# maruscia/fastkmer

Hardware: AMD Instinct MI355X
Metric: input bases/sec (whole node), k=28 short reads, 1/2/4/8 GPUs (higher is better)
Workload: dtype u64; 1 GPU; BASELINE configs[1]: k=28 m=10 x=3 B=2048, 1 GB synthetic 100 bp reads per GPU; k=28, m=10, x=3, B=2048, useHT=0, sequenceType=0, fasta_bytes_per_gpu=999999906, bases_per_gpu=877192900, parallelism=one GPU

## Files before the change

fastkmer_amd/__init__.py:

```python
from __future__ import annotations

import ctypes
import dataclasses
import os
import re

import numpy as np

_PKG = os.path.dirname(os.path.abspath(__file__))
LIB_PATH = os.environ.get("FASTKMER_LIB") or os.path.join(_PKG, "lib", "libfastkmer.so")
CLI_PATH = os.path.join(_PKG, "bin", "fastkmer-cli")
HEADER_PATH = os.path.join(os.path.dirname(_PKG), "include", "fastkmer.h")

FK_OK = 0
ERRORS = {-1: "FK_E_INVALID", -2: "FK_E_STATE", -3: "FK_E_DEVICE", -4: "FK_E_NOMEM", -5: "FK_E_IO",
          -6: "FK_E_RANGE", -7: "FK_E_COMM"}
ABI_VERSION = 3


class FastKmerError(RuntimeError):
    def __init__(self, code: int, message: str):
        super().__init__(f"{ERRORS.get(code, code)}: {message}")
        self.code = code

# ... 74 lines not shown
        "fk_synth_record_bytes": (U64, [I32]),
        "fk_synth_fasta_host": (ctypes.c_int, [P, U64, U64, I32, U64, U64, ctypes.c_double, ctypes.c_double]),
        "fk_create": (ctypes.c_int, [ctypes.POINTER(fk_config), ctypes.POINTER(P)]),
        "fk_destroy": (None, [P]),
        "fk_last_error": (ctypes.c_char_p, []),
        "fk_set_stream": (ctypes.c_int, [P, P]),
        "fk_ingest": (ctypes.c_int, [P, ctypes.c_char_p, SZ, ctypes.c_int]),
        "fk_ingest_device": (ctypes.c_int, [P, P, SZ, ctypes.c_int]),
        "fk_ingest_reserve": (ctypes.c_int, [P, U64]),
        "fk_split_bytes": (ctypes.c_int, [ctypes.c_char_p, I32, I32, I32, I32, P, SZ, ctypes.POINTER(SZ)]),
        "fk_ingest_file_range": (ctypes.c_int, [P, ctypes.c_char_p, I32, I32, U64]),
        "fk_set_input_format": (ctypes.c_int, [P, I32, I32, I32]),
        "fk_input_format": (ctypes.c_int, [P, ctypes.POINTER(I32), ctypes.POINTER(I32), ctypes.POINTER(I32)]),
        "fk_fastq_info": (ctypes.c_int, [P, P]),
        "fk_debug_fastq_ms": (ctypes.c_int, [P, ctypes.POINTER(ctypes.c_double), ctypes.POINTER(U64)]),
        "fk_fastq_frontier": (ctypes.c_int, [ctypes.c_char_p, SZ, ctypes.POINTER(SZ)]),
        "fk_split_bytes_fastq": (ctypes.c_int, [ctypes.c_char_p, I32, I32, P, SZ, ctypes.POINTER(SZ)]),
        "fk_synth_fasta_device": (ctypes.c_int, [P, U64, U64, I32, U64, U64, ctypes.c_double, ctypes.c_double]),
        "fk_synth_fasta_to_device": (ctypes.c_int, [P, U64, U64, I32, U64, U64, ctypes.c_double, ctypes.c_double]),
        "fk_map": (ctypes.c_int, [P, P]),
        "fk_record_bytes": (SZ, [P]),
        "fk_map_emit": (ctypes.c_int, [P, P, U64]),
        "fk_reduce": (ctypes.c_int, [P, P, U64]),
        "fk_set_grouped_emit": (ctypes.c_int, [P, ctypes.c_int32]),
        "fk_grouped_parts_per_rank": (ctypes.c_int32, [P]),
        "fk_map_part_counts": (ctypes.c_int, [P, P, P]),
        "fk_reduce_grouped": (ctypes.c_int, [P, P, U64, P, P, ctypes.c_int32, ctypes.c_int32]),
        "fk_finish": (ctypes.c_int, [P]),
        "fk_num_bins": (I32, [P]),
        "fk_bin_sizes": (ctypes.c_int, [P, P]),
        "fk_get_bin": (ctypes.c_int, [P, I32, P, P, SZ, ctypes.POINTER(SZ)]),
        "fk_write_bins": (ctypes.c_int, [P, ctypes.c_char_p]),
        "fk_get_stats": (ctypes.c_int, [P, ctypes.POINTER(fk_stats)]),
        "fk_kmer_bin": (ctypes.c_int, [ctypes.POINTER(fk_config), P, P]),
        "fk_query": (ctypes.c_int, [P, P, SZ, P, P]),
        "fk_query_device": (ctypes.c_int, [P, P, SZ, P, P]),
        "fk_query_sequence": (ctypes.c_int, [P, ctypes.c_char_p, SZ, P, SZ, ctypes.POINTER(SZ)]),
        "fk_reads_csr": (ctypes.c_int, [ctypes.c_char_p, SZ, I32, I32, I32, P, SZ, P, SZ, ctypes.POINTER(SZ),
                                        ctypes.POINTER(SZ)]),
        "fk_read_counts_device": (ctypes.c_int, [P, P, P, SZ, P, P]),
        "fk_read_counts": (ctypes.c_int, [P, P, P, SZ, P, P]),
        "fk_read_stats_of_counts_device": (ctypes.c_int, [P, P, P, P, SZ, ctypes.c_uint32, ctypes.c_uint32, P]),
        "fk_read_stats_device": (ctypes.c_int, [P, P, P, SZ, ctypes.c_uint32, ctypes.c_uint32, P, SZ, P]),
        "fk_read_stats": (ctypes.c_int, [P, P, P, SZ, ctypes.c_uint32, ctypes.c_uint32, P]),
        "fk_read_stats_scratch_bytes": (SZ, [SZ]),
        "fk_spectrum": (ctypes.c_int, [P, P, SZ, P]),
        "fk_spectrum_device": (ctypes.c_int, [P, P, SZ, P]),
        "fk_bin_sizes_range": (ctypes.c_int, [P, ctypes.c_uint32, ctypes.c_uint32, P]),
        "fk_get_bin_range": (ctypes.c_int, [P, I32, ctypes.c_uint32, ctypes.c_uint32, P, P, SZ,
                                            ctypes.POINTER(SZ)]),
        "fk_write_bins_range": (ctypes.c_int, [P, ctypes.c_char_p, ctypes.c_uint32, ctypes.c_uint32]),
        "fk_compare": (ctypes.c_int, [P, P, P, SZ, SZ]),
        "fk_compare_device": (ctypes.c_int, [P, P, P, SZ, SZ]),
        "fk_bin_sizes_joined": (ctypes.c_int, [P, P, ctypes.c_uint32, ctypes.c_uint32, ctypes.c_uint32,
                                               ctypes.c_uint32, P]),
        "fk_get_bin_joined": (ctypes.c_int, [P, P, I32, ctypes.c_uint32, ctypes.c_uint32, ctypes.c_uint32,
                                             ctypes.c_uint32, P, P, P, SZ, ctypes.POINTER(SZ)]),
        "fk_map_bin_kmers": (ctypes.c_int, [P, P]),
        "fk_lpt_owners": (ctypes.c_int, [P, I32, I32, P]),
        "fk_set_bin_owners": (ctypes.c_int, [P, P, P]),
        "fk_bin_owners": (ctypes.c_int, [P, P]),
        "fk_signature_slots": (U64, [P]),
        "fk_signature_counts": (ctypes.c_int, [P, P, U64]),
        "fk_write_bin_signatures": (ctypes.c_int, [P, P, U64, ctypes.c_char_p]),
        "fk_find_bin_signatures": (ctypes.c_int, [P, ctypes.c_char_p]),
        "fk_comm_unique_id": (ctypes.c_int, [P]),
        "fk_comm_init": (ctypes.c_int, [P, P]),
        "fk_comm_init_local": (ctypes.c_int, [P, I32]),
        "fk_comm_transport": (ctypes.c_char_p, [P]),
        "fk_comm_allreduce_u64": (ctypes.c_int, [P, P, SZ]),
        "fk_balance_bins": (ctypes.c_int, [P, ctypes.c_char_p, SZ]),
        "fk_balance_bins_file": (ctypes.c_int, [P, ctypes.c_char_p, I32, I32, ctypes.c_double]),
        "fk_exchange_plan": (ctypes.c_int, [I32, I32, P, P, U64, P, P, P, P, P]),
        "fk_debug_map_cycles": (ctypes.c_int, [P, I32]),
        "fk_debug_comm_hold": (ctypes.c_int, [P, I32]),
        "fk_debug_comm_release": (ctypes.c_int, [P]),
        "fk_debug_comm_held": (ctypes.c_int, [P]),
        "fk_debug_fingerprint_bits": (ctypes.c_int, [I32, I32]),
        "fk_debug_wave_count": (ctypes.c_int, [I32, I32, I32, ctypes.c_uint32, ctypes.c_uint32, I32, P,
                                               ctypes.c_uint32, P, P, P]),
        "fk_debug_wave_count_w": (ctypes.c_int, [I32, I32, I32, ctypes.c_uint32, ctypes.c_uint32, I32, P,
                                                 ctypes.c_uint32, P, P, P]),
        "fk_debug_fold_stats": (ctypes.c_int, [P, P]),
    }
    for name, (res, args) in sig.items():
        fn = getattr(L, name)
        fn.restype = res
        fn.argtypes = args
    if L.fk_abi_version() != ABI_VERSION:
        raise RuntimeError(f"{LIB_PATH} has ABI version {L.fk_abi_version()}, this binding mirrors {ABI_VERSION}: "
                           "rebuild it (python -m fastkmer_amd.build)")
    _lib = L
    return L


def _check(rc: int) -> None:
    if rc != FK_OK:
        raise FastKmerError(rc, lib().fk_last_error().decode(errors="replace"))


def make_config(k: int, m: int, x: int = 3, B: int = 2048, use_ht: bool = False, sequence_type: int = 0,
                write: bool = False, n_ranks: int = 1, rank: int = 0, device: int = -1) -> fk_config:
    c = fk_config()
    lib().fk_config_init(ctypes.byref(c))
    c.k, c.m, c.x, c.B = k, m, x, B
    c.use_ht, c.sequence_type, c.write = int(bool(use_ht)), sequence_type, int(bool(write))
    c.n_ranks, c.rank, c.device = n_ranks, rank, device
    return c


def validate(**kw) -> None:
    c = make_config(**kw)
    _check(lib().fk_config_validate(ctypes.byref(c)))


def clamped_bins(m: int, B: int) -> int:
    return lib().fk_clamped_bins(m, B)


def record_bytes_for_k(k: int) -> int:
    return lib().fk_record_bytes_for_k(k)


def synth_fasta(n_reads: int, read_len: int = 100, genome_len: int = 1_000_000, seed: int = 0x5EED,
                err_rate: float = 0.002, n_rate: float = 0.0005, first_read: int = 0) -> bytes:
    L = lib()
    nb = n_reads * L.fk_synth_record_bytes(read_len)
    buf = ctypes.create_string_buffer(max(nb, 1))
    _check(L.fk_synth_fasta_host(buf, first_read, n_reads, read_len, genome_len, seed, err_rate, n_rate))
    return buf.raw[:nb]


def synth_fasta_to_device(ptr: int, n_reads: int, read_len: int = 100, genome_len: int = 1_000_000,
                          seed: int = 0x5EED, err_rate: float = 0.002, n_rate: float = 0.0005,
                          first_read: int = 0) -> int:
    L = lib()
    _check(L.fk_synth_fasta_to_device(ctypes.c_void_p(ptr), first_read, n_reads, read_len, genome_len, seed,
                                      err_rate, n_rate))
    return n_reads * L.fk_synth_record_bytes(read_len)


def split_bytes(path: str, world: int, rank: int, k: int, sequence_type: int = 0) -> bytes:
    L = lib()
    n = ctypes.c_size_t()
    p = os.fsencode(path)
    _check(L.fk_split_bytes(p, world, rank, k, sequence_type, None, 0, ctypes.byref(n)))
    buf = ctypes.create_string_buffer(max(n.value, 1))
    _check(L.fk_split_bytes(p, world, rank, k, sequence_type, buf, n.value, ctypes.byref(n)))
    return buf.raw[:n.value]


FORMATS = {"fasta": 0, "fastq": 1}


def split_bytes_fastq(path: str, world: int, rank: int) -> bytes:
    L = lib()
    n = ctypes.c_size_t()
    p = os.fsencode(path)
    _check(L.fk_split_bytes_fastq(p, world, rank, None, 0, ctypes.byref(n)))
    buf = ctypes.create_string_buffer(max(n.value, 1))
    _check(L.fk_split_bytes_fastq(p, world, rank, buf, n.value, ctypes.byref(n)))
    return buf.raw[:n.value]


def fastq_frontier(buf: bytes) -> int:
    raw = bytes(buf)
# ... 412 lines not shown
    def read_stats(self, bases_or_text, offsets=None, min_count: int = 1, max_count: int | None = None,
                   input_format: str = "fasta", min_quality: int = 0, quality_offset: int = 33) -> np.ndarray:
        if offsets is None:
            bases_or_text, offsets = reads_csr(bases_or_text, input_format, min_quality, quality_offset)
        b, o = _csr_arrays(bases_or_text, offsets)
        hi = MAX_COUNT if max_count is None else int(max_count)
        if not (0 <= int(min_count) <= MAX_COUNT and 0 <= hi <= MAX_COUNT):
            raise ValueError("min_count / max_count are 32-bit counts")
        stats = np.zeros(o.size - 1, dtype=READ_STAT_DTYPE)
        _check(lib().fk_read_stats(self._h, b.ctypes.data, o.ctypes.data, o.size - 1, int(min_count), hi,
                                   stats.ctypes.data))
        return stats

    def read_counts_ptr(self, d_bases: int, d_offsets: int, n_reads: int, d_counts: int, d_valid: int = 0) -> None:
        _check(lib().fk_read_counts_device(self._h, ctypes.c_void_p(d_bases), ctypes.c_void_p(d_offsets), n_reads,
                                           ctypes.c_void_p(d_counts), ctypes.c_void_p(d_valid) if d_valid else None))

    def read_stats_ptr(self, d_bases: int, d_offsets: int, n_reads: int, d_scratch: int, scratch_bytes: int,
                       d_stats: int, min_count: int = 1, max_count: int | None = None) -> None:
        _check(lib().fk_read_stats_device(self._h, ctypes.c_void_p(d_bases), ctypes.c_void_p(d_offsets), n_reads,
                                          int(min_count), MAX_COUNT if max_count is None else int(max_count),
                                          ctypes.c_void_p(d_scratch), scratch_bytes, ctypes.c_void_p(d_stats)))

    def read_stats_of_counts_ptr(self, d_counts: int, d_valid: int, d_offsets: int, n_reads: int, d_stats: int,
                                 min_count: int = 1, max_count: int | None = None) -> None:
        _check(lib().fk_read_stats_of_counts_device(self._h, ctypes.c_void_p(d_counts),
                                                    ctypes.c_void_p(d_valid) if d_valid else None,
                                                    ctypes.c_void_p(d_offsets), n_reads, int(min_count),
                                                    MAX_COUNT if max_count is None else int(max_count),
                                                    ctypes.c_void_p(d_stats)))

    def bin_dict(self, b: int, min_count: int = 1, max_count: int | None = None) -> dict:
        keys, counts = self.get_bin(b, min_count, max_count)
        return dict(zip(decode_keys(keys, self.k), (int(c) for c in counts)))

    def all_dict(self) -> dict:
        sizes = self.bin_sizes()
        return {b: self.bin_dict(b) for b in np.nonzero(sizes)[0].tolist()}

    def bin_text(self, b: int, min_count: int = 1, max_count: int | None = None) -> str:
        keys, counts = self.get_bin(b, min_count, max_count)
        lines = [f"{s}\t{int(c)}\n" for s, c in zip(decode_keys(keys, self.k), counts)]
        if not lines and _count_range(min_count, max_count) is not None:
            return ""
        return "".join(lines) + ("" if self.use_ht else "EOF")

    def write_bins(self, out_dir: str, min_count: int = 1, max_count: int | None = None) -> None:
        rg = _count_range(min_count, max_count)
        if rg is None:
            _check(lib().fk_write_bins(self._h, out_dir.encode()))
        else:
            _check(lib().fk_write_bins_range(self._h, out_dir.encode(), rg[0], rg[1]))

    def signature_counts(self, out=None):
        import torch
        n = lib().fk_signature_slots(self._h)
        if out is None:
            out = torch.empty(n, dtype=torch.int64, device=self._torch_device())
        if out.numel() < n or out.dtype != torch.int64 or not out.is_cuda or not out.is_contiguous():
            raise ValueError(f"signature counts need a contiguous device int64 tensor of {n} entries")
        _check(lib().fk_signature_counts(self._h, ctypes.c_void_p(out.data_ptr()), out.numel()))
        return out

    def write_bin_signatures(self, counts, out_dir: str) -> None:
        _check(lib().fk_write_bin_signatures(self._h, ctypes.c_void_p(counts.data_ptr()), counts.numel(),
                                             out_dir.encode()))

    def _torch_device(self):
        import torch
        return torch.device("cuda", self._device if self._device >= 0 else torch.cuda.current_device())

    def stats(self) -> dict:
        st = fk_stats()
        _check(lib().fk_get_stats(self._h, ctypes.byref(st)))
        return {n: getattr(st, n) for n, _ in fk_stats._fields_}

    def fold_stats(self) -> dict:
        out = (ctypes.c_uint64 * 4)()
        _check(lib().fk_debug_fold_stats(self._h, out))
        return {"pieces_folded": int(out[0]), "entries_in": int(out[1]), "entries_out": int(out[2]),
                "sample_ratio": int(out[3]) / 1e6 if out[3] else None}


def debug_wave_count(keys: np.ndarray, k: int, F: int, c0: int, c1: int, slots: int, device: int = 0,
                     weighted: bool = False):
    kw = 1 if k <= 32 else 2
    keys = np.ascontiguousarray(keys, dtype=np.uint64).reshape(-1, kw)
    n = len(keys)
    ok = np.zeros(n * kw, dtype=np.uint64)
    oc = np.zeros(n, dtype=np.uint32)
    nout = ctypes.c_uint32(0)
    fn = lib().fk_debug_wave_count_w if weighted else lib().fk_debug_wave_count
    _check(fn(device, k, F, c0, c1, slots, keys.ctypes.data, n, ok.ctypes.data, oc.ctypes.data, ctypes.byref(nout)))
    u = nout.value
    return (ok[:u] if kw == 1 else ok[:2 * u].reshape(-1, 2)), oc[:u]


def comm_unique_id() -> bytes:
    buf = ctypes.create_string_buffer(COMM_ID_BYTES)
    _check(lib().fk_comm_unique_id(buf))
    return buf.raw


def comm_init_local(counters) -> None:
    arr = (ctypes.c_void_p * len(counters))(*[c._h.value for c in counters])
    _check(lib().fk_comm_init_local(arr, len(counters)))


def exchange_plan(sent, received, record_bytes: int):
    snd = np.ascontiguousarray(sent, dtype=np.uint64)
    rcv = np.ascontiguousarray(received, dtype=np.uint64)
    if snd.ndim != 2 or snd.shape != rcv.shape or snd.shape[1] % 2 != 1:
        raise ValueError("sent / received must be [n_ranks, 2 * parts + 1] arrays of one shape")
    n, parts = snd.shape[0], (snd.shape[1] - 1) // 2
    so, sb, ro, rb = (np.zeros(n, dtype=np.uint64) for _ in range(4))
    fin = ctypes.c_int32(0)
    _check(lib().fk_exchange_plan(n, parts, snd.ctypes.data, rcv.ctypes.data, record_bytes, so.ctypes.data,
                                  sb.ctypes.data, ro.ctypes.data, rb.ctypes.data, ctypes.byref(fin)))
    return so, sb, ro, rb, bool(fin.value)


def lpt_owners(sizes, n_ranks: int) -> np.ndarray:
    sz = np.ascontiguousarray(sizes, dtype=np.uint64)
    owner = np.zeros(len(sz), dtype=np.int32)
    _check(lib().fk_lpt_owners(sz.ctypes.data, len(sz), n_ranks, owner.ctypes.data))
    return owner


def execute_job(configuration: TestConfiguration, input_format: str = "fasta", min_quality: int = 0,
                quality_offset: int = 33) -> KmerCounter:
    with open(configuration.dataset, "rb") as f:
        data = f.read()
    kc = KmerCounter(configuration.k, configuration.m, configuration.x, configuration.max_b,
                     configuration.useHT, configuration.sequenceType, input_format=input_format,
                     min_quality=min_quality, quality_offset=quality_offset)
    kc.ingest(data)
    kc.finish()
    if configuration.write:
        kc.write_bins(configuration.outputDir)
    return kc


def execute_find_bin_signatures_job(configuration: TestConfiguration):
    with open(configuration.dataset, "rb") as f:
        data = f.read()
    with KmerCounter(configuration.k, configuration.m, configuration.x, configuration.max_b,
                     configuration.useHT, configuration.sequenceType) as kc:
        kc.ingest(data)
        counts = kc.signature_counts()
        kc.write_bin_signatures(counts, configuration.outputDir)
    return counts
```

fastkmer_amd/csrc/fk_api.cpp:

```cpp
#include <errno.h>
#include <fcntl.h>
#include <unistd.h>
#include <stdarg.h>
#include <stdio.h>
#include <string.h>
#include <sys/stat.h>

#include <unordered_map>
#include <chrono>
#include <cstdlib>
#include <cstring>
#include <thread>

#include "fk_ctx.h"
#include "fk_split.h"

static thread_local std::string g_err;
int fk::set_err(int code, const char *fmt, ...) {
    char buf[1024];
    va_list ap;
    va_start(ap, fmt);
    vsnprintf(buf, sizeof(buf), fmt, ap);
    va_end(ap);
    g_err = buf;
// ... 151 lines not shown
                           c->k, c->m, c->x, clamp_bins(c->m, c->B), c->sequence_type);
    if (n < 0 || (size_t)n >= cap) return set_err(FK_E_RANGE, "output buffer too small (%d bytes needed)", n + 1);
    return FK_OK;
}

FK_EXPORT size_t fk_record_bytes_for_k(int32_t k) { return k <= 32 ? 16 : 24; }

FK_EXPORT uint64_t fk_synth_record_bytes(int32_t read_len) { return (uint64_t)read_len + 14; }

static SynthParams make_synth(uint64_t first_read, uint64_t n_reads, int32_t read_len, uint64_t genome_len,
                              uint64_t seed, double err_rate, double n_rate) {
    SynthParams p;
    p.first_read = first_read;
    p.n_reads = n_reads;
    p.genome_len = genome_len;
    p.seed = seed;
    p.read_len = (uint32_t)read_len;
    p.rec_bytes = (uint32_t)read_len + 14;
    const double two64 = 18446744073709551616.0;
    p.err_thresh = (uint64_t)(err_rate * two64 * 0.999999);
    p.n_thresh = (uint64_t)(n_rate * two64 * 0.999999);
    return p;
}

FK_EXPORT int fk_synth_fasta_host(uint8_t *out, uint64_t first_read, uint64_t n_reads, int32_t read_len,
                                  uint64_t genome_len, uint64_t seed, double err_rate, double n_rate) {
    if (!out || read_len < 1 || genome_len < 1) return set_err(FK_E_INVALID, "bad synth arguments");
    const SynthParams p = make_synth(first_read, n_reads, read_len, genome_len, seed, err_rate, n_rate);
    const uint64_t nb = n_reads * p.rec_bytes;
    for (uint64_t i = 0; i < nb; ++i) out[i] = synth_byte(p, i);
    return FK_OK;
}


FK_EXPORT int fk_create(const fk_config *cfg, fk_ctx **out) {
    if (!out) return set_err(FK_E_INVALID, "null output pointer");
    *out = nullptr;
    FK_TRY(fk_config_validate(cfg));
    int ndev = 0;
    hipError_t e = hipGetDeviceCount(&ndev);
    if (e != hipSuccess || ndev <= 0) {
        (void)hipGetLastError();
        return set_err(FK_E_DEVICE, "no HIP device available (%s): the k-mer counter runs on MI355X only",
                       hipGetErrorString(e));
    }
    fk_ctx *c = new fk_ctx();
    c->cfg = *cfg;
    c->Bc = clamp_bins(cfg->m, cfg->B);
    c->G = (uint32_t)cfg->n_ranks;
    c->nlb = (uint32_t)((c->Bc - cfg->rank + (int)c->G - 1) / (int)c->G);
    if (cfg->rank >= c->Bc) c->nlb = 0;
    c->W = cfg->k <= 32 ? 2 : 3;
    c->KW = cfg->k <= 32 ? 1 : 2;
    c->fm = make_fastmod((uint32_t)c->Bc);
    auto env = [](const char *name) -> const char * {
        const char *v = getenv(name);
        return v && v[0] ? v : nullptr;
    };
    if (const char *v = env("FASTKMER_PIECE_BYTES")) {
        c->piece_bytes = std::max(1ull << 16, strtoull(v, nullptr, 10));
        c->piece_bytes_set = true;
    }
    if (const char *v = env("FASTKMER_PIECE_CUTS")) {
        c->st_cuts.clear();
        c->xst_cuts.clear();
        for (const char *q = v; *q;) {
            char *e = nullptr;
            const double f = strtod(q, &e);
            if (e == q) break;
            if (f > 0.0 && f < 1.0 && c->st_cuts.size() < STAGE_MAXP - 1) c->st_cuts.push_back(f), c->xst_cuts.push_back(f);
            c->cuts_env = true;
            q = *e == ',' ? e + 1 : e;
        }
    }
    if (const char *v = env("FASTKMER_INGEST_SEG")) c->ingest_seg = std::max(1ull << 16, strtoull(v, nullptr, 10));
    if (const char *v = env("FASTKMER_DEBUG_LARGE_BUCKETS")) c->force_large = v[0] == '1';
    if (const char *v = env("FASTKMER_DEBUG_CELL_TARGET")) c->cell_target = (uint32_t)atoi(v);
    if (const char *v = env("FASTKMER_DEBUG_MID_PARTS")) c->mid_parts = atoi(v);
    if (const char *v = env("FASTKMER_DEBUG_SPLIT_RETRY")) c->split_retry = v[0] == '1';
    if (const char *v = env("FASTKMER_DEBUG_SPECTRUM_WIDE")) c->spectrum_wide = v[0] == '1';
    if (const char *v = env("FASTKMER_FOLD")) c->fold_mode = std::clamp(atoi(v), 0, 2);
    if (const char *v = env("FASTKMER_DEBUG_FOLD_WMAX"))
        c->fold_wmax = (uint32_t)std::clamp(atoi(v), 1, (int)WKEY_WMAX);
    if (const char *v = env("FASTKMER_X2_L1")) c->x2_l1 = atoi(v);
    if (const char *v = env("FASTKMER_FUSED")) c->fused = atoi(v);
#ifdef FK_PROBES
    if (const char *v = env("FASTKMER_DEBUG_PHASE")) c->dbg_phase = atoi(v);
    if (const char *v = env("FASTKMER_FUSED_PROBE")) c->fused_probe = atoi(v);
    if (const char *v = env("FASTKMER_SPLIT_MAP")) c->split_map = atoi(v);
#endif
    if (cfg->device >= 0) {
        if (cfg->device >= ndev) {
            delete c;
            return set_err(FK_E_DEVICE, "device %d out of range (%d devices)", cfg->device, ndev);
        }
        c->device = cfg->device;
    } else {
        (void)hipGetDevice(&c->device);
    }
    DeviceGuard dg_(c->device);
    {
        int cur = -1;
        if (hipGetDevice(&cur) != hipSuccess || cur != c->device) {
            (void)hipGetLastError();
            delete c;
            return set_err(FK_E_DEVICE, "cannot select device %d", c->device);
        }
    }
    e = hipStreamCreateWithFlags(&c->stream, hipStreamNonBlocking);
    if (e != hipSuccess) {
        delete c;
        return set_err(FK_E_DEVICE, "hipStreamCreate: %s", hipGetErrorString(e));
    }
    c->own_stream = true;
    e = hipStreamCreateWithFlags(&c->copy_stream, hipStreamNonBlocking);
    if (e == hipSuccess) e = hipEventCreateWithFlags(&c->seg_ev, hipEventDisableTiming);
    if (e == hipSuccess) e = hipStreamCreateWithFlags(&c->xstage, hipStreamNonBlocking);
    if (e == hipSuccess) e = hipEventCreateWithFlags(&c->xstage_ev, hipEventDisableTiming);
    if (e == hipSuccess) {
        int least = 0, greatest = 0;
        if (hipDeviceGetStreamPriorityRange(&least, &greatest) == hipSuccess)
            e = hipStreamCreateWithPriority(&c->tier_side, hipStreamNonBlocking, greatest);
        else
            e = hipStreamCreateWithFlags(&c->tier_side, hipStreamNonBlocking);
    }
    for (int i = 0; i < 4 && e == hipSuccess; ++i) e = hipEventCreateWithFlags(&c->side_ev[i], hipEventDisableTiming);
    for (int i = 0; i < 2 && e == hipSuccess; ++i) e = hipEventCreate(&c->h2d_ev[i]);
    if (e != hipSuccess) {
        fk_destroy(c);
        return set_err(FK_E_DEVICE, "copy stream / events: %s", hipGetErrorString(e));
    }
    for (auto &ev : c->ev) {
        e = hipEventCreate(&ev);
        if (e != hipSuccess) {
            fk_destroy(c);
            return set_err(FK_E_DEVICE, "hipEventCreate: %s", hipGetErrorString(e));
        }
    }
    e = hipEventCreateWithFlags(&c->tier_ev, hipEventDisableTiming);
    if (e == hipSuccess) e = hipEventCreateWithFlags(&c->pin_up_ev, hipEventDisableTiming);
    if (e == hipSuccess) e = hipEventCreateWithFlags(&c->cmp_ev, hipEventDisableTiming);
    if (e != hipSuccess) {
        fk_destroy(c);
        return set_err(FK_E_DEVICE, "hipEventCreate: %s", hipGetErrorString(e));
    }
    for (auto &ev : c->st_ev) {
        e = hipEventCreate(&ev);
        if (e != hipSuccess) {
            fk_destroy(c);
            return set_err(FK_E_DEVICE, "hipEventCreate: %s", hipGetErrorString(e));
        }
    }
    *out = c;
    return FK_OK;
}

FK_EXPORT void fk_destroy(fk_ctx *c) {
    if (!c) return;
    DeviceGuard dg_(c->device);
    if (c->hold_flag) __atomic_store_n(c->hold_flag, 1u, __ATOMIC_RELEASE);
    if (c->copy_stream) (void)hipStreamSynchronize(c->copy_stream);
    if (c->stream) (void)hipStreamSynchronize(c->stream);
    if (c->xstage) (void)hipStreamSynchronize(c->xstage);
    if (c->tier_side) (void)hipStreamSynchronize(c->tier_side);
    DevBuf *bufs[] = {&c->fasta_own, &c->tile_last_nl, &c->tile_off,
                      &c->npos_dev, &c->codes, &c->valid, &c->records, &c->counters, &c->sig_status, &c->sig_kmers, &c->tcnt, &c->rec_hdr, &c->rec_pos, &c->rec_code, &c->tstat, &c->map_vslots,
                      &c->precs, &c->chunks, &c->bin_chunk_begin, &c->hpieces, &c->hpiece_first, &c->hpiece_tot, &c->chunk_nk, &c->grp_table,
                      &c->chunk_base, &c->lp, &c->scratch,
                      &c->cell_total, &c->cell_base, &c->flags, &c->flag_scan, &c->buckets, &c->keys,
                      &c->out_keys, &c->out_counts, &c->bucket_unique, &c->dense_off, &c->dense_keys,
                      &c->dense_counts, &c->bin_off, &c->misc, &c->tier_list, &c->mid, &c->sc_total,
                      &c->sp_base, &c->sp_keys, &c->sp_subs, &c->sp_par, &c->sp_fb, &c->mid_fb};
    for (DevBuf *b : bufs) release(*b);
    c->vw.release_all();
    release(c->fq_ws);
    release(c->fq_info);
    for (auto &e : c->fq_evs)
        if (e) (void)hipEventDestroy(e);
    c->fq_pin.release();
    for (int i = 0; i < 2; ++i) {
        if (c->pinned[i]) (void)hipHostFree(c->pinned[i]);
        if (c->pin_ev[i]) (void)hipEventDestroy(c->pin_ev[i]);
    }
    if (c->comm_stream) (void)hipStreamSynchronize(c->comm_stream);
    delete c->comm;
    c->comm = nullptr;
    c->pin_up.release();
    c->pin_down.release();
    c->pin_tier.release();
    c->fold_pin.release();
    c->file_pin[0].release();
    c->file_pin[1].release();
    if (c->tier_ev) (void)hipEventDestroy(c->tier_ev);
    if (c->pin_up_ev) (void)hipEventDestroy(c->pin_up_ev);
    if (c->cmp_ev) (void)hipEventDestroy(c->cmp_ev);
    if (c->hold_flag) (void)hipHostFree(c->hold_flag);
    release(c->xsend);
    release(c->xrecv);
    for (auto &e : c->xev)
        if (e) (void)hipEventDestroy(e);
    for (auto &e : c->seg_evs)
        if (e) (void)hipEventDestroy(e);
    for (auto &e : c->map_evs)
        if (e) (void)hipEventDestroy(e);
    if (c->emit_ev) (void)hipEventDestroy(c->emit_ev);
    if (c->comm_stream) (void)hipStreamDestroy(c->comm_stream);
    if (c->xstage) (void)hipStreamSynchronize(c->xstage), (void)hipStreamDestroy(c->xstage);
    if (c->xstage_ev) (void)hipEventDestroy(c->xstage_ev);
    if (c->ws_x.ptr) (void)hipFree(c->ws_x.ptr);
    c->dest.release_all();
    c->part.release_all();
    c->binhist.release_all();
    release(c->d_owner);
    release(c->d_local);
    if (c->ws.ptr) (void)hipFree(c->ws.ptr);
    for (auto &ev : c->ev)
        if (ev) (void)hipEventDestroy(ev);
    for (auto &ev : c->st_ev)
        if (ev) (void)hipEventDestroy(ev);
    for (int p = 0; p < STAGE_MAXP; ++p) release(c->st_keys[p]), release(c->st_cb[p]);
    release(c->st_total);
    release(c->fold_cnt), release(c->fold_cb), release(c->fold_io);
    release(c->piece_starts);
    if (c->seg_ev) (void)hipEventDestroy(c->seg_ev);
    for (auto &ev : c->h2d_ev)
        if (ev) (void)hipEventDestroy(ev);
    if (c->tier_side) (void)hipStreamSynchronize(c->tier_side), (void)hipStreamDestroy(c->tier_side);
    for (auto &ev : c->side_ev)
        if (ev) (void)hipEventDestroy(ev);
    if (c->copy_stream) (void)hipStreamDestroy(c->copy_stream);
    if (c->own_stream && c->stream) (void)hipStreamDestroy(c->stream);
    delete c;
}

FK_EXPORT int fk_set_stream(fk_ctx *c, void *s) {
    if (!c) return set_err(FK_E_INVALID, "null ctx");
    DeviceGuard dg_(c->device);
    if (c->own_stream && c->stream) {
        (void)hipStreamSynchronize(c->stream);
        (void)hipStreamDestroy(c->stream);
    }
    c->stream = (hipStream_t)s;
    c->own_stream = false;
    return FK_OK;
}

FK_EXPORT size_t fk_record_bytes(const fk_ctx *c) { return c ? (size_t)c->W * 8 : 0; }
FK_EXPORT int32_t fk_num_bins(const fk_ctx *c) { return c ? c->Bc : 0; }

static void reset_results(fk_ctx *c) {
    c->mapped = false;
    c->have_result = false;
    c->gapped = c->dense_ready = false;
    c->distinct = 0;
    c->h_bin_off.clear();
}

static float ev_ms(hipEvent_t a, hipEvent_t b) {
    float ms = 0.f;
    if (hipEventElapsedTime(&ms, a, b) != hipSuccess) {
        (void)hipGetLastError();
        return 0.f;
    }
    return ms;
}

constexpr size_t PIN_CHUNK = 32ull << 20;

static int grow_keep(DevBuf &b, size_t bytes, size_t keep, hipStream_t s) {
    if (b.bytes >= bytes) return FK_OK;
    DevBuf g;
    FK_TRY(ensure(g, std::max<size_t>(bytes, 2 * b.bytes)));
    if (keep && b.p) HIP_TRY(hipMemcpyAsync(g.p, b.p, std::min(keep, b.bytes), hipMemcpyDeviceToDevice, s));
    HIP_TRY(hipStreamSynchronize(s));
    release(b);
    b = g;
    return FK_OK;
}


FK_EXPORT int fk_set_input_format(fk_ctx *c, int32_t format, int32_t min_quality, int32_t quality_offset) {
    if (!c) return set_err(FK_E_INVALID, "null ctx");
    if (c->job_open) return set_err(FK_E_STATE, "fk_set_input_format inside a job (after its first fk_ingest)");
    if (format != FK_FORMAT_FASTA && format != FK_FORMAT_FASTQ) return set_err(FK_E_INVALID, "unknown input format %d", format);
    if (quality_offset != 33 && quality_offset != 64)
        return set_err(FK_E_INVALID, "quality_offset must be 33 or 64, got %d", quality_offset);
    if (min_quality < 0 || min_quality > 93) return set_err(FK_E_INVALID, "min_quality must be in 0..93, got %d", min_quality);
    if (format == FK_FORMAT_FASTQ && c->cfg.sequence_type != 0)
        return set_err(FK_E_INVALID, "FASTQ input needs sequence_type 0 (short reads)");
    c->in_format = format;
    c->fq_min_q = min_quality;
    c->fq_q_off = quality_offset;
    return FK_OK;
}

FK_EXPORT int fk_input_format(const fk_ctx *c, int32_t *format, int32_t *min_quality, int32_t *quality_offset) {
    if (!c) return set_err(FK_E_INVALID, "null ctx");
    if (format) *format = c->in_format;
    if (min_quality) *min_quality = c->fq_min_q;
    if (quality_offset) *quality_offset = c->fq_q_off;
    return FK_OK;
}

FK_EXPORT int fk_fastq_info(fk_ctx *c, uint64_t out[3]) {
    if (!c || !out) return set_err(FK_E_INVALID, "null argument");
// ... 64 lines not shown
                                end > FQ_LOOK ? end - FQ_LOOK : 0);
        if (f == end) f = c->fq_done;
    }
    FK_TRY(fq_normalise(c, nullptr, c->fq_done, f, final_));
    c->fq_done = f;
    *limit = f;
    return FK_OK;
}

static int fq_finish_pending(fk_ctx *c, uint64_t n) {
    if (!c->fq_job || c->fq_done >= n) return FK_OK;
    FK_TRY(fq_normalise(c, nullptr, c->fq_done, n, true));
    c->fq_done = n;
    c->fq_tail.clear();
    return FK_OK;
}

static int fq_info_queue(fk_ctx *c) {
    if (c->fq_job && c->fq_launched)
        HIP_TRY(hipMemcpyAsync(c->fq_pin.p, c->fq_info.p, 32, hipMemcpyDeviceToHost, c->stream));
    return FK_OK;
}
static int fq_info_read(fk_ctx *c) {
    if (!c->fq_job) return FK_OK;
    const uint64_t *h = c->fq_pin.as<uint64_t>();
    const bool any = c->fq_launched;
    c->fq_out[0] = any ? h[0] : 0;
    c->fq_out[1] = any ? h[1] : 0;
    c->fq_out[2] = any && h[2] ? ~h[2] : UINT64_MAX;
    c->fq_have_info = true;
    if (any && h[3])
        return set_err(FK_E_INVALID, "FASTQ: more than one line per 4 bytes over a range of the input (the line index overflowed)");
    if (c->fq_out[2] != UINT64_MAX)
        return set_err(FK_E_INVALID, "FASTQ record %llu is malformed (no '@' or '+' line, quality and sequence of "
                                     "different lengths, or the input ends inside it)", (unsigned long long)c->fq_out[2]);
    return FK_OK;
}

static bool premap_eligible(const fk_ctx *c) {
    return c->fused && map_fused_supported(c->cfg.k, c->cfg.m, (uint32_t)c->Bc);
}

constexpr uint64_t MAP_VSLOT_TILES = 32768;
static int map_vslots_reserve(fk_ctx *c, uint64_t ntiles) {
    if (!map_split(c)) return FK_OK;
    return ensure(c->map_vslots, std::min(ntiles, MAP_VSLOT_TILES) * map_fused_vslot() * 4);
}
static int map_launch(fk_ctx *c, const uint8_t *fa, uint64_t n, int more, uint64_t t0, uint64_t nt, hipStream_t s) {
    const uint64_t cap = map_split(c) ? c->map_vslots.bytes / ((uint64_t)map_fused_vslot() * 4) : 0;
    for (uint64_t b = 0; b < nt;) {
        const uint64_t m = cap ? std::min(cap, nt - b) : nt - b;
        HIP_TRY(launch_map_fused(FUSED_NT, c->cfg.k, c->cfg.m, fa, n, more, t0 + b, m, c->fm,
                                 c->rec_hdr.as<uint32_t>(), c->rec_pos.as<uint16_t>(), c->rec_code.as<uint32_t>(),
                                 c->tcnt.as<uint32_t>(), c->tstat.as<uint32_t>(), c->counters.as<unsigned long long>(),
                                 s, fused_probe(c), cap ? c->map_vslots.as<uint32_t>() : nullptr));
        b += m;
    }
    return FK_OK;
}

static int premap_launch(fk_ctx *c, uint64_t landed, bool final_) {
    const uint64_t tile = fm_tile_bytes(FUSED_NT), span = fm_span_bytes(FUSED_NT);
    const uint64_t end = final_ ? (landed + tile - 1) / tile : (landed >= span ? (landed - span) / tile + 1 : 0);
    if (end <= c->pm_tiles) return FK_OK;
    if (c->tcnt.bytes < end * 4 || c->tstat.bytes < end * 8 || c->rec_hdr.bytes < end * map_fused_tcap() * 4 ||
        c->rec_pos.bytes < end * map_fused_tcap() * 2 || c->rec_code.bytes < end * map_fused_cslot() * 4)
        return set_err(FK_E_STATE, "streamed map: %llu tiles exceed the reserved record slots",
                       (unsigned long long)end);
    hipStream_t s = c->stream;
    if (c->pm_tiles == 0) HIP_TRY(hipEventRecord(c->ev[10], s));
    FK_TRY(map_launch(c, c->d_fasta, landed, final_ ? 0 : 1, c->pm_tiles, end - c->pm_tiles, s));
    c->pm_tiles = end;
    if (final_) HIP_TRY(hipEventRecord(c->ev[11], s));
    return FK_OK;
}

static int xch_maybe_piece(fk_ctx *c);
static int local_maybe_piece(fk_ctx *c, uint64_t tiles, hipEvent_t mapped);
static void xch_reset(fk_ctx *c);
static void pieces_reset(fk_ctx *c);

static int comm_fail(fk_ctx *c, int rc);
static int note_held(fk_ctx *c, int rc);

static int ingest_impl(fk_ctx *c, const uint8_t *fasta, size_t n, int last) {
    if (!fasta && n) return set_err(FK_E_INVALID, "null argument");
    DeviceGuard dg_(c->device);
    if (c->d_fasta && c->d_fasta != c->fasta_own.as<uint8_t>()) {
        if (c->dev_open) return set_err(FK_E_STATE, "fk_ingest appending to an fk_ingest_device input");
        c->d_fasta = nullptr;
    }
    hipStream_t s = c->stream, cs = c->copy_stream;
    const bool fresh = c->ingest_fresh || !c->d_fasta;
    if (fresh) {
        c->n_fasta = 0;
        c->ingest_fresh = false;
        if (c->comm) {
            if (c->xch.open) return set_err(FK_E_STATE, "fk_ingest: the previous job's exchange is unfinished (fk_finish)");
            FK_TRY(comm_sync(c, c->comm_stream));
            xch_reset(c);
        }
        FK_TRY(comm_sync(c, c->xstage));
        HIP_TRY(hipStreamSynchronize(c->tier_side));
        HIP_TRY(hipStreamSynchronize(s));
        pieces_reset(c);
        c->pm_active = premap_eligible(c);
        c->pm_tiles = 0;
        c->pm_last_seen = false;
        FK_TRY(fq_begin_job(c, c->in_format == FK_FORMAT_FASTQ));
    } else if (c->pm_last_seen) {
        c->pm_active = false;
    }
    const uint64_t have = c->n_fasta, need = have + n;
    if (c->fasta_own.bytes < need) {
        HIP_TRY(hipStreamSynchronize(cs));
        FK_TRY(grow_keep(c->fasta_own, need, have, s));
    }
    c->d_fasta = c->fasta_own.as<uint8_t>();
    const bool fq = c->fq_job;
    if (fq) FK_TRY(ensure(c->fq_ws, fastq_ws_bytes(std::min<uint64_t>(n, 4 * c->ingest_seg) + (1u << 20))));
    if (c->pm_active) {
        const uint64_t tiles = (need + fm_tile_bytes(FUSED_NT) - 1) / fm_tile_bytes(FUSED_NT) + 1;
        if (c->tcnt.bytes < tiles * 4) FK_TRY(grow_keep(c->tcnt, tiles * 4, c->tcnt.bytes, s));
        if (c->tstat.bytes < tiles * 8) FK_TRY(grow_keep(c->tstat, tiles * 8, c->tstat.bytes, s));
        const uint64_t hdr_need = tiles * map_fused_tcap() * 4, pos_need = tiles * map_fused_tcap() * 2;
        const uint64_t code_need = tiles * map_fused_cslot() * 4;
        if (c->rec_hdr.bytes < hdr_need) FK_TRY(grow_keep(c->rec_hdr, hdr_need, c->rec_hdr.bytes, s));
        if (c->rec_pos.bytes < pos_need) FK_TRY(grow_keep(c->rec_pos, pos_need, c->rec_pos.bytes, s));
        if (c->rec_code.bytes < code_need) FK_TRY(grow_keep(c->rec_code, code_need, c->rec_code.bytes, s));
        FK_TRY(map_vslots_reserve(c, tiles));
        if (fresh) {
            FK_TRY(ensure(c->counters, 64));
            HIP_TRY(hipMemsetAsync(c->counters.p, 0, 64, s));
        }
    }
    uint8_t *dst = c->fasta_own.as<uint8_t>() + have;
    hipPointerAttribute_t attr{};
    const bool pinned = hipPointerGetAttributes(&attr, fasta) == hipSuccess && attr.type == hipMemoryTypeHost;
    (void)hipGetLastError();
    if (!pinned && n)
        for (int i = 0; i < 2; ++i)
            if (!c->pinned[i]) {
                HIP_TRY(hipHostMalloc(&c->pinned[i], PIN_CHUNK, hipHostMallocDefault));
                HIP_TRY(hipEventCreateWithFlags(&c->pin_ev[i], hipEventDisableTiming));
                HIP_TRY(hipEventRecord(c->pin_ev[i], cs));
            }
    const bool pieces = c->comm && c->pm_active;
    if (pieces && fresh) {
        c->xch.expect_bytes = last ? n : c->reserve_bytes;
        constexpr uint64_t XCH_STEPS = 10;
        constexpr uint64_t XCH_MIN = 64ull << 20;
        if (!c->piece_bytes_set)
            c->piece_bytes = c->xch.expect_bytes
                                 ? std::min<uint64_t>(1ull << 30, std::max<uint64_t>(XCH_MIN, c->xch.expect_bytes / XCH_STEPS))
                                 : 1ull << 30;
    }
    if (fresh) {
        c->job_bytes = last ? n : c->reserve_bytes;
        c->reserve_bytes = 0;
    }
    HIP_TRY(hipEventRecord(c->h2d_ev[0], cs));
    if (pinned) {
        const size_t seg = c->ingest_seg;
        size_t big = seg * std::clamp<size_t>((n / 16 + seg / 2) / seg, 1, 4);
        if (pieces) big = std::min(big, std::max(seg, (size_t)c->piece_bytes / 4 / seg * seg));
        const size_t nseg = (n + seg - 1) / seg;
        const size_t small_from = n - std::min(n, std::max<size_t>(n / 10, 4 * seg));
        auto seg_len = [&](size_t off) { return std::min(off < small_from ? big : seg, n - off); };
        while ((c->pm_active || fq) && c->seg_evs.size() < nseg) {
            hipEvent_t e = nullptr;
            HIP_TRY(hipEventCreateWithFlags(&e, hipEventDisableTiming));
            c->seg_evs.push_back(e);
        }
        size_t off = 0;
        for (size_t i = 0; off < n; ++i) {
            const size_t len = seg_len(off);
            HIP_TRY(hipMemcpyAsync(dst + off, fasta + off, len, hipMemcpyHostToDevice, cs));
            if (c->pm_active || fq) HIP_TRY(hipEventRecord(c->seg_evs[i], cs));
            off += len;
        }
        HIP_TRY(hipEventRecord(c->h2d_ev[1], cs));
        while (!pieces && c->pm_active && c->map_evs.size() < nseg) {
            hipEvent_t e = nullptr;
            HIP_TRY(hipEventCreateWithFlags(&e, hipEventDisableTiming));
            c->map_evs.push_back(e);
        }
        c->seg_tiles.clear();
        off = 0;
        for (size_t i = 0; (c->pm_active || fq) && off < n; ++i) {
            off += seg_len(off);
            HIP_TRY(hipStreamWaitEvent(s, c->seg_evs[i], 0));
            uint64_t limit = have + off;
            if (fq) FK_TRY(fq_advance(c, fasta, have, off, last && off == n, &limit));
            if (!c->pm_active) continue;
            FK_TRY(premap_launch(c, limit, last && off == n));
            if (pieces) {
                FK_TRY(xch_maybe_piece(c));
            } else {
                HIP_TRY(hipEventRecord(c->map_evs[i], s));
                c->seg_tiles.push_back(c->pm_tiles);
            }
        }
        for (size_t i = 0; !pieces && c->pm_active && i < c->seg_tiles.size(); ++i)
            FK_TRY(local_maybe_piece(c, c->seg_tiles[i], c->map_evs[i]));
    } else {
        size_t off = 0;
        for (int i = 0; off < n; ++i) {
            const size_t len = std::min(PIN_CHUNK, n - off);
            HIP_TRY(hipEventSynchronize(c->pin_ev[i & 1]));
            memcpy(c->pinned[i & 1], fasta + off, len);
            HIP_TRY(hipMemcpyAsync(dst + off, c->pinned[i & 1], len, hipMemcpyHostToDevice, cs));
            HIP_TRY(hipEventRecord(c->pin_ev[i & 1], cs));
            off += len;
            if (c->pm_active || fq) {
                HIP_TRY(hipEventRecord(c->seg_ev, cs));
                HIP_TRY(hipStreamWaitEvent(s, c->seg_ev, 0));
                uint64_t limit = have + off;
                if (fq) FK_TRY(fq_advance(c, fasta, have, off, last && off == n, &limit));
                if (!c->pm_active) continue;
                FK_TRY(premap_launch(c, limit, last && off == n));
                if (pieces) {
                    FK_TRY(xch_maybe_piece(c));
                } else {
                    HIP_TRY(hipEventRecord(c->seg_ev, s));
                    FK_TRY(local_maybe_piece(c, c->pm_tiles, c->seg_ev));
                }
            }
        }
        HIP_TRY(hipEventRecord(c->h2d_ev[1], cs));
    }
    if (fq) {
        uint64_t limit = 0;
        if (last && n == 0) FK_TRY(fq_advance(c, fasta, have, 0, true, &limit));
        const uint64_t tb = have - c->fq_tail.size();
        std::vector<uint8_t> tail;
        if (c->fq_done < have) tail.assign(c->fq_tail.begin() + (c->fq_done - tb), c->fq_tail.end());
        const uint64_t from = c->fq_done > have ? c->fq_done - have : 0;
        if (from < n) tail.insert(tail.end(), fasta + from, fasta + n);
        c->fq_tail.swap(tail);
    }
    if (c->pm_active && last) {
        c->pm_last_seen = true;
        if (n == 0) FK_TRY(premap_launch(c, need, true));
    }
    HIP_TRY(hipStreamSynchronize(cs));
    c->ms_h2d = ev_ms(c->h2d_ev[0], c->h2d_ev[1]);
    c->n_fasta = need;
    reset_results(c);
    return FK_OK;
}
// ... 476 lines not shown
    return FK_OK;
}

FK_EXPORT int fk_set_bin_owners(fk_ctx *c, const int32_t *owner, uint64_t *send_counts) {
    if (!c || !owner) return set_err(FK_E_INVALID, "null argument");
    DeviceGuard dg_(c->device);
    if (c->comm && c->xch.open) return set_err(FK_E_STATE, "fk_set_bin_owners inside a job's exchange");
    for (int32_t b = 0; b < c->Bc; ++b)
        if (owner[b] < 0 || (uint32_t)owner[b] >= c->G)
            return set_err(FK_E_INVALID, "owner[%d] = %d is not a rank of %u", b, owner[b], c->G);
    hipStream_t s = c->stream;
    c->h_owner.assign(owner, owner + c->Bc);
    c->h_bin_lbin.assign(c->Bc, ~0u);
    c->h_lbin_bin.clear();
    for (int32_t b = 0; b < c->Bc; ++b)
        if (owner[b] == c->cfg.rank) {
            c->h_bin_lbin[b] = (uint32_t)c->h_lbin_bin.size();
            c->h_lbin_bin.push_back(b);
        }
    c->nlb = (uint32_t)c->h_lbin_bin.size();
    const uint64_t ntab = (uint64_t)REC_BIN_MASK + 1;
    FK_TRY(ensure(c->d_owner, ntab * 4));
    FK_TRY(ensure(c->d_local, ntab * 4));
    HIP_TRY(hipMemsetAsync(c->d_owner.p, 0xff, ntab * 4, s));
    HIP_TRY(hipMemsetAsync(c->d_local.p, 0xff, ntab * 4, s));
    HIP_TRY(hipMemcpyAsync(c->d_owner.p, c->h_owner.data(), (uint64_t)c->Bc * 4, hipMemcpyHostToDevice, s));
    HIP_TRY(hipMemcpyAsync(c->d_local.p, c->h_bin_lbin.data(), (uint64_t)c->Bc * 4, hipMemcpyHostToDevice, s));
    c->custom_owners = true;
    c->have_result = false;
    if (c->grouped) {
        FK_TRY(build_group_table(c));
        if (c->mapped) FK_TRY(grouped_part_counts(c));
    } else if (c->mapped) {
        c->send_counts.assign(c->G, 0);
        if (c->G == 1) {
            c->send_counts[0] = c->nrec;
        } else if (c->nrec) {
            FK_TRY(part_count(c->dest, map_src(c), 0, c->G, owner_table(c), c->G, c->ws, s));
            HIP_TRY(hipMemcpyAsync(c->send_counts.data(), c->dest.rec.p, c->G * 8, hipMemcpyDeviceToHost, s));
        }
    }
    HIP_TRY(hipStreamSynchronize(s));
    if (send_counts)
        for (uint32_t r = 0; r < c->G; ++r) send_counts[r] = c->mapped ? c->send_counts[r] : 0;
    return FK_OK;
}

FK_EXPORT int fk_bin_owners(const fk_ctx *c, int32_t *owner) {
    if (!c || !owner) return set_err(FK_E_INVALID, "null argument");
    for (int32_t b = 0; b < c->Bc; ++b) owner[b] = c->custom_owners ? c->h_owner[b] : (int32_t)((uint32_t)b % c->G);
    return FK_OK;
}


static bool staged_ok(const fk_ctx *c) {
#ifdef FK_PROBES
    if (c->dbg_phase != 99) return false;
#endif
    return c->cfg.k <= 63 && !c->force_large;
}

static SortedPlan sorted_plan(const fk_ctx *c, uint64_t max_bin_kmers) {
    SortedPlan pl;
    const int k = c->cfg.k;
    const uint32_t cap = 2048;
    const bool tiered = staged_ok(c);
    const bool two_level = c->cfg.k <= 63;
    constexpr uint64_t CELL_TARGET64 = 512;
    const uint64_t target = c->cell_target ? c->cell_target
                                           : (c->KW == 2 && tiered ? WAVE128_BUCKET_CAP / 2
                                                                   : two_level ? CELL_TARGET64 : cap / 4);
    int F = 1;
    while (F < MAX_FINE_BITS && ((uint64_t)1 << F) * target < max_bin_kmers) ++F;
    if (!two_level) F = std::min(F, MAX_FINE_BITS - 1);
    F = std::min(F, 2 * k);
    const uint32_t wave_cap = c->KW == 1 ? WAVE_BUCKET_CAP : WAVE128_BUCKET_CAP;
    const int F2 = std::min(F, std::max(5, std::min(6, F - 8))), F1 = F - F2;
    pl.F = F, pl.F2 = F2, pl.F1 = F1, pl.tiered = tiered, pl.two_level = two_level, pl.cap = cap, pl.wave_cap = wave_cap;
    pl.max_bin = max_bin_kmers;
    return pl;
}

static int sorted_expand(fk_ctx *c, StreamWs on, hipStream_t cut, const SortedPlan &pl, uint32_t nchunks,
                         uint64_t total_kmers, DevBuf &keys, DevBuf &cell_base_buf) {
    hipStream_t s = on.s;
    const int k = c->cfg.k;
    const int F = pl.F, F2 = pl.F2, F1 = pl.F1;
    const bool two_level = pl.two_level;
    const uint32_t ncell = 1u << F;
    const uint64_t ncell_all = (uint64_t)c->nlb << F;
    FK_TRY(ensure(keys, total_kmers * 8 * c->KW));
    FK_TRY(ensure(c->cell_total, ncell_all * 8));
    FK_TRY(ensure(cell_base_buf, (ncell_all + 1) * 8));
    uint64_t *const cell_base = cell_base_buf.as<uint64_t>();
    if (two_level) {
        const uint64_t nsc_all = (uint64_t)c->nlb << F1;
        FK_TRY(ensure(c->lp, ((uint64_t)nchunks << F1) * 4));
        FK_TRY(ensure(c->sc_total, nsc_all * 8));
        constexpr double HIST_PIECES = 1024.0;
        std::vector<uint32_t> pieces, first;
        bool split = false;
        if (nchunks && c->h_bcb.size() == (size_t)c->nlb + 1) {
            for (uint32_t lb = 0; lb < c->nlb; ++lb) {
                const uint32_t cb = c->h_bcb[lb], ce = c->h_bcb[lb + 1], nc = ce - cb;
                const uint32_t P = std::max(1u, std::min(nc, (uint32_t)(HIST_PIECES * nc / nchunks + 0.5)));
                const uint32_t f = (uint32_t)(pieces.size() / 4);
                for (uint32_t q = 0; q < P; ++q) {
                    pieces.insert(pieces.end(), {lb, cb + nc * q / P, cb + nc * (q + 1) / P, P == 1 ? 1u : 0u});
                    first.push_back(f);
                }
                split |= P > 1;
            }
        }
        if (split) {
            const uint32_t np = (uint32_t)first.size();
            FK_TRY(ensure(c->hpieces, (uint64_t)np * 16));
            FK_TRY(ensure(c->hpiece_first, (uint64_t)np * 4));
            FK_TRY(ensure(c->hpiece_tot, ((uint64_t)np << F1) * 4));
            HIP_TRY(hipMemcpyAsync(c->hpieces.p, pieces.data(), (uint64_t)np * 16, hipMemcpyHostToDevice, s));
            HIP_TRY(hipMemcpyAsync(c->hpiece_first.p, first.data(), (uint64_t)np * 4, hipMemcpyHostToDevice, s));
            HIP_TRY(hipMemsetAsync(c->cell_total.p, 0, ncell_all * 8, s));
            HIP_TRY(launch_expand_hist_pieces(c->KW, c->rsrc, c->chunks.as<Chunk>(), c->hpieces.as<uint4>(),
                                              c->hpiece_first.as<uint32_t>(), np, k, F, F2,
                                              c->cell_total.as<uint64_t>(), c->lp.as<uint32_t>(),
                                              c->hpiece_tot.as<uint32_t>(), s));
            HIP_TRY(hipStreamSynchronize(s));
        } else {
            HIP_TRY(launch_expand_hist_bin(c->KW, c->rsrc, c->chunks.as<Chunk>(), c->bin_chunk_begin.as<uint32_t>(),
                                           c->nlb, k, F, F2, c->cell_total.as<uint64_t>(), c->lp.as<uint32_t>(), s));
        }
    } else {
        FK_TRY(ensure(c->lp, (uint64_t)nchunks * ncell * 4));
        HIP_TRY(launch_expand_hist(c->W, c->rsrc, c->chunks.as<Chunk>(), nchunks, k, F,
                                   c->lp.as<uint32_t>(), s));
        HIP_TRY(launch_cell_prefix(c->bin_chunk_begin.as<uint32_t>(), c->nlb, F, c->lp.as<uint32_t>(),
                                   c->cell_total.as<uint64_t>(), s));
    }
    HIP_TRY(scan_excl_sum_u64(c->cell_total.as<uint64_t>(), cell_base, ncell_all, cell_base + ncell_all, *on.ws, s));
    if (cut) HIP_TRY(hipEventRecord(c->side_ev[2], s));
    if (two_level) {
        FK_TRY(ensure(c->mid, total_kmers * 8 * c->KW));
        HIP_TRY(launch_expand_two_level(c->KW, c->rsrc, c->chunks.as<Chunk>(), nchunks, c->nlb, k, F,
                                        F2, c->lp.as<uint32_t>(), cell_base, c->mid.as<uint64_t>(),
                                        keys.as<uint64_t>(), s, c->x2_l1, total_kmers));
    } else {
        HIP_TRY(launch_expand_scatter(c->W, c->rsrc, c->chunks.as<Chunk>(), nchunks, k, F,
                                      c->lp.as<uint32_t>(), cell_base, keys.as<uint64_t>(), s));
    }
    return FK_OK;
}

struct CountBufs {
    DevBuf *flags, *flag_scan, *buckets, *bucket_unique, *tier_list, *piece_starts, *out_counts;
};
static CountBufs main_bufs(fk_ctx *c) {
    return CountBufs{&c->flags, &c->flag_scan, &c->buckets, &c->bucket_unique, &c->tier_list, &c->piece_starts,
                     &c->out_counts};
}

struct BucketCount {
    fk_ctx *c;
    BucketSrc src;
    CountBufs B;
    DevBuf &okb;
    int k;
    uint32_t cap;
    bool ordered;
    StreamWs s, cut, heavy;
    uint64_t nbuckets = 0;
    uint32_t *lists = nullptr;
    uint32_t ntier[2] = {0, 0};
    uint64_t listed_keys = 0;
    bool mid_wave = false;
    uint32_t *mid_fb = nullptr, *fbB = nullptr, *fbG = nullptr;
    uint32_t nmidfb = 0, nfbB = 0, nfbG = 0;

    const Bucket *buckets() const { return B.buckets->as<Bucket>(); }
    uint64_t *out_keys() const { return okb.as<uint64_t>(); }
    uint32_t *out_counts() const { return B.out_counts->as<uint32_t>(); }
    uint64_t *unique() const { return B.bucket_unique->as<uint64_t>(); }
    uint32_t mid_cap() const { return c->KW == 1 ? WAVE_MID_CAP : WAVE128_MID_CAP; }
    unsigned int *mid_fb_count() const { return c->misc.as<unsigned int>() + 11; }
};

static hipError_t launch_wave_tier(const BucketCount &t, hipStream_t s) {
    if (t.c->KW == 1)
        return launch_bucket_count64_wave(t.src, t.buckets(), t.nbuckets, t.k, t.out_keys(), t.out_counts(), t.unique(),
                                          nullptr, s, t.ordered);
    return launch_bucket_count128_wave(t.src, t.buckets(), t.nbuckets, t.k, t.out_keys(), t.out_counts(), t.unique(), s,
                                       t.ordered);
}
static hipError_t launch_wave_mid(const BucketCount &t, const uint32_t *list, uint32_t n, hipStream_t s) {
    if (t.c->KW == 1)
        return launch_bucket_count64_wave_mid(t.src, t.buckets(), list, n, t.k, t.out_keys(), t.out_counts(), t.unique(),
                                              s, t.ordered);
    return launch_bucket_count128_wave_mid(t.src, t.buckets(), list, n, t.k, t.out_keys(), t.out_counts(), t.unique(), s,
                                           t.ordered);
}
static hipError_t launch_split(const BucketCount &t, const uint32_t *l1, uint32_t nl, SubBucket *subs,
                               unsigned int *counts, uint32_t *fb, hipStream_t s) {
    fk_ctx *c = t.c;
    return launch_bucket_split64(t.src, t.buckets(), t.lists, 0, l1, nl, c->sp_base.as<uint64_t>(),
                                 c->sp_keys.as<uint64_t>(), subs, c->sp_par.as<SplitParent>(), counts, fb, fb + nl,
                                 t.cap, t.k, t.src.F, s, c->split_retry);
}
static hipError_t launch_split(const BucketCount &t, const uint32_t *l1, uint32_t nl, SubBucket128 *subs,
                               unsigned int *counts, uint32_t *fb, hipStream_t s) {
    fk_ctx *c = t.c;
    return launch_bucket_split128(t.src, t.buckets(), l1, nl, c->sp_base.as<uint64_t>(), c->sp_keys.as<uint64_t>(), subs,
                                  c->sp_par.as<SplitParent>(), counts, fb, fb + nl, t.cap, t.k, t.src.F, s,
                                  c->split_retry);
}
static hipError_t launch_sub_count_seq(const BucketCount &t, const uint32_t *l1, uint32_t nl, const SubBucket *subs,
                                       hipStream_t s) {
    return launch_sub_count64_seq(t.buckets(), l1, nl, t.c->sp_par.as<SplitParent>(), subs, t.c->sp_keys.as<uint64_t>(),
                                  t.k, t.src.weighted, t.out_keys(), t.out_counts(), t.unique(), s, t.ordered);
}
static hipError_t launch_sub_count_seq(const BucketCount &t, const uint32_t *l1, uint32_t nl, const SubBucket128 *subs,
                                       hipStream_t s) {
    return launch_sub_count128_seq(t.buckets(), l1, nl, t.c->sp_par.as<SplitParent>(), subs, t.c->sp_keys.as<uint64_t>(),
                                   t.out_keys(), t.out_counts(), t.unique(), s, t.ordered);
}

static int block_tier(const BucketCount &t, const uint32_t *list, uint32_t n, hipStream_t s) {
    fk_ctx *c = t.c;
    if (c->KW == 1)
        HIP_TRY(launch_bucket_count64(t.src, t.buckets(), n, t.k, t.out_keys(), t.out_counts(), t.unique(),
                                      c->misc.as<unsigned long long>() + 1, t.cap, 99, list, s, 0));
    else
        HIP_TRY(launch_bucket_sort(2, t.src, t.buckets(), n, t.k, t.out_keys(), t.out_counts(), t.unique(),
                                   c->misc.as<unsigned long long>() + 1, t.cap, list, s, 0));
// ... 463 lines not shown
    HIP_TRY(hipMemcpy(c->grp_table.p, table.data(), (uint64_t)c->Bc * 4, hipMemcpyHostToDevice));
    return FK_OK;
}

FK_EXPORT int32_t fk_grouped_parts_per_rank(const fk_ctx *c) { return c && c->grouped ? (int32_t)c->grp_nlb : 0; }

FK_EXPORT int fk_map_part_counts(fk_ctx *c, uint64_t *records, uint64_t *kmers) {
    if (!c || !records || !kmers) return set_err(FK_E_INVALID, "null argument");
    if (!c->grouped || !c->mapped) return set_err(FK_E_STATE, "fk_map_part_counts needs fk_set_grouped_emit and fk_map");
    std::copy(c->grp_rec.begin(), c->grp_rec.end(), records);
    std::copy(c->grp_kmer.begin(), c->grp_kmer.end(), kmers);
    return FK_OK;
}

static int reduce_ranges(fk_ctx *c, const uint64_t *d_recv, uint64_t nrecv,
                         const std::vector<std::vector<std::pair<uint64_t, uint64_t>>> &ranges,
                         const std::vector<uint64_t> &bkm, double t0) {
    std::vector<Chunk> chunks;
    std::vector<uint32_t> bcb;
    build_chunks(c->nlb, ranges, chunks, bcb);
    FK_TRY(upload_chunks(c, c->stream, chunks, bcb));
    HIP_TRY(hipEventRecord(c->ev[5], c->stream));
    c->rsrc = d_recv;
    return reduce_tail(c, nrecv, chunks, bcb, bkm, t0);
}

FK_EXPORT int fk_reduce_grouped(fk_ctx *c, const void *d_recv, uint64_t nrecv, const uint64_t *seg_records,
                                const uint64_t *seg_kmers, int32_t nseg, int32_t parts_per_seg) {
    if (!c) return set_err(FK_E_INVALID, "null ctx");
    DeviceGuard dg_(c->device);
    if (nrecv && !d_recv) return set_err(FK_E_INVALID, "null receive buffer");
    if (nseg < 0 || parts_per_seg < 0 || (nseg && (!seg_records || !seg_kmers)))
        return set_err(FK_E_INVALID, "bad segment table");
    const double t0 = now_ms();
    hipStream_t s = c->stream;
    c->have_result = false;
    const uint32_t nlb = c->nlb;
    if ((uint32_t)parts_per_seg < nlb) return set_err(FK_E_INVALID, "%d parts per segment < %u local bins",
                                                      parts_per_seg, nlb);
    HIP_TRY(hipEventRecord(c->ev[4], s));
    std::vector<std::vector<std::pair<uint64_t, uint64_t>>> ranges(nlb);
    std::vector<uint64_t> bkm(nlb, 0);
    uint64_t off = 0;
    for (int32_t sg = 0; sg < nseg; ++sg) {
        for (int32_t lb = 0; lb < parts_per_seg; ++lb) {
            const uint64_t n = seg_records[(uint64_t)sg * parts_per_seg + lb];
            if (n && (uint32_t)lb >= nlb) return set_err(FK_E_INVALID, "records for local bin %d of %u", lb, nlb);
            if (n) {
                ranges[lb].push_back({off, off + n});
                bkm[lb] += seg_kmers[(uint64_t)sg * parts_per_seg + lb];
            }
            off += n;
        }
    }
    if (off != nrecv)
        return set_err(FK_E_INVALID, "segment table holds %llu records, buffer %llu", (unsigned long long)off,
                       (unsigned long long)nrecv);
    return reduce_ranges(c, (const uint64_t *)d_recv, nrecv, ranges, bkm, t0);
}


static void pieces_reset(fk_ctx *c) {
    c->st_np = 0;
    c->st_cut = 0;
    c->st_kmers = 0;
    c->pieces_void = false;
    c->tiles_counted = 0;
    c->segs_counted = 0;
    c->fold_decided = c->fold_on = false;
    c->fold_sample_ppm = 0;
    c->fold_in = 0;
    c->fold_pieces.clear();
}

static uint32_t stage_maxp(const fk_ctx *c) { return c->KW == 2 ? (uint32_t)STAGE_MAXP128 : (uint32_t)STAGE_MAXP; }
static const std::vector<double> &local_cuts(const fk_ctx *c) {
    if (!c->cuts_env && c->KW == 1 && c->job_bytes >= (4ull << 30) && STAGE_MAXP >= 5) return c->st_cuts5;
    return c->st_cuts;
}

static bool staged_eligible(const fk_ctx *c) { return staged_ok(c) && c->G == 1 && !c->comm; }

static int staged_expand_chunks(fk_ctx *c, StreamWs on, hipStream_t cut, uint32_t nchunks,
                                const std::vector<uint64_t> &bkm, double frac) {
    hipStream_t s = on.s;
    const uint32_t p = c->st_np;
    uint64_t pk = 0, maxb = 0;
    for (uint64_t v : bkm) pk += v, maxb = std::max(maxb, v);
    if (pk == 0) return FK_OK;
    if (p == 0) {
        const double scale = frac > 0.0 ? std::max(1.0, 1.0 / frac) : 2.0;
        c->st_plan = sorted_plan(c, (uint64_t)((double)maxb * scale));
        if (!c->st_plan.tiered || !c->st_plan.two_level)
            return set_err(FK_E_STATE, "staged pieces need the tiered two-level count");
    }
    SortedPlan pl = c->st_plan;
    HIP_TRY(hipEventRecord(c->st_ev[4 * p + 2], s));
    FK_TRY(sorted_expand(c, on, cut, pl, nchunks, pk, c->st_keys[p], c->st_cb[p]));
    const uint64_t ncell_all = (uint64_t)c->nlb << c->st_plan.F;
    FK_TRY(ensure(c->st_total, ncell_all * 8));
    if (cut) {
        HIP_TRY(hipStreamWaitEvent(cut, c->side_ev[2], 0));
        HIP_TRY(launch_add_u64(c->st_total.as<uint64_t>(), c->cell_total.as<uint64_t>(), ncell_all, p == 0, cut));
    } else {
        HIP_TRY(launch_add_u64(c->st_total.as<uint64_t>(), c->cell_total.as<uint64_t>(), ncell_all, p == 0, s));
    }
    HIP_TRY(hipEventRecord(c->st_ev[4 * p + 3], s));
    c->st_kmers += pk;
    c->st_np = p + 1;
    htrace("staged: piece expanded");
    return FK_OK;
}

static int staged_expand(fk_ctx *c, StreamWs on, hipStream_t cut, const RecSrc &src, double frac) {
    const uint32_t p = c->st_np;
    if (p >= stage_maxp(c)) return set_err(FK_E_STATE, "more than %u staged pieces", stage_maxp(c));
    uint64_t nrecv = 0;
    std::vector<Chunk> chunks;
    std::vector<uint32_t> bcb;
    std::vector<uint64_t> bkm;
    FK_TRY(partition_src(c, on, src, nrecv, chunks, bcb, bkm, c->st_ev[4 * p], c->st_ev[4 * p + 1]));
    return staged_expand_chunks(c, on, cut, (uint32_t)chunks.size(), bkm, frac);
}

static int staged_count(fk_ctx *c, hipStream_t cut) {
    const double t0 = now_ms();
    const StreamWs on = c->main_on();
    hipStream_t s = on.s;
    const SortedPlan pl = c->st_plan;
    const uint32_t nlb = c->nlb;
    const uint64_t ncell_all = (uint64_t)nlb << pl.F;
    HIP_TRY(hipEventRecord(c->ev[6], s));
    std::swap(c->cell_total, c->st_total);
    FK_TRY(ensure(c->cell_base, (ncell_all + 1) * 8));
    const hipStream_t cs = cut ? cut : s;
    if (cut) HIP_TRY(hipStreamWaitEvent(cut, c->side_ev[2], 0));
    HIP_TRY(scan_excl_sum_u64(c->cell_total.as<uint64_t>(), c->cell_base.as<uint64_t>(), ncell_all,
                              c->cell_base.as<uint64_t>() + ncell_all, *on.ws, cs));
    BucketSrc src{nullptr, pl.F};
    src.np = (int)c->st_np;
    src.weighted = !c->fold_pieces.empty();
    for (uint32_t p = 0; p < c->st_np; ++p) {
        src.pk[p] = c->st_keys[p].as<uint64_t>();
        src.pcb[p] = c->st_cb[p].as<uint64_t>();
    }
    FK_TRY(sorted_count(c, on, cut, pl, src, c->st_kmers));
    HIP_TRY(hipEventRecord(c->ev[7], s));
    FK_TRY(read_bin_offsets(c, s));
    htrace("staged: bin offsets read");
    double mp = 0.0, mx = 0.0;
    for (uint32_t p = 0; p < c->st_np; ++p) {
        mp += ev_ms(c->st_ev[4 * p], c->st_ev[4 * p + 1]);
        mx += ev_ms(c->st_ev[4 * p + 2], c->st_ev[4 * p + 3]);
    }
    c->stats.ms_partition = mp;
    c->stats.ms_count = mx + ev_ms(c->ev[6], c->ev[7]);
    c->stats.pieces_counted = c->st_np;
    count_done(c, c->nrec, t0);
    return FK_OK;
}

static bool local_piece_due(const fk_ctx *c, uint64_t tiles) {
    constexpr uint64_t MIN_PIECE = 256ull << 20;
    if (c->st_np >= stage_maxp(c) - 1) return false;
    const uint64_t tile = fm_tile_bytes(FUSED_NT);
    if (c->job_bytes && !c->piece_bytes_set) {
        const std::vector<double> &cuts = local_cuts(c);
        if (c->job_bytes < 2 * MIN_PIECE || c->st_cut >= cuts.size()) return false;
        const uint64_t end = (uint64_t)(cuts[c->st_cut] * (double)c->job_bytes);
        return tiles * tile >= end && (tiles - c->tiles_counted) * tile >= MIN_PIECE / 2;
    }
    return c->st_np < 3 && (tiles - c->tiles_counted) * tile >= c->piece_bytes;
}

static bool fold_eligible(const fk_ctx *c) {
    return c->fold_mode != 0 && c->KW == 1 && 2 * c->cfg.k <= WKEY_MAX_BITS && staged_eligible(c);
}

constexpr uint32_t FOLD_SAMPLE_STRIDE = 61;
constexpr uint64_t FOLD_SAMPLE_MAX = 4096;
constexpr uint64_t FOLD_MAX_PPM = 600000;
static int fold_decide(fk_ctx *c, StreamWs on, uint32_t p) {
    c->fold_decided = true;
    c->fold_on = c->fold_mode == 2;
    if (c->fold_mode != 1) return FK_OK;
    const SortedPlan &pl = c->st_plan;
    FK_TRY(ensure(c->fold_io, 16));
    const uint64_t nsc = (uint64_t)c->nlb << pl.F1;
    const uint32_t stride = (uint32_t)std::max<uint64_t>(FOLD_SAMPLE_STRIDE, (nsc / FOLD_SAMPLE_MAX) | 1ull);
    HIP_TRY(hipMemsetAsync(c->fold_io.p, 0, 16, on.s));
    HIP_TRY(launch_fold_sample(c->st_keys[p].as<uint64_t>(), c->st_cb[p].as<uint64_t>(), c->nlb, c->cfg.k, pl.F, pl.F2,
                               c->fold_wmax, stride, c->fold_io.as<unsigned long long>(), on.s));
    uint64_t io[2] = {0, 0};
    HIP_TRY(hipMemcpyAsync(io, c->fold_io.p, 16, hipMemcpyDeviceToHost, on.s));
    HIP_TRY(hipStreamSynchronize(on.s));
    c->fold_sample_ppm = io[0] ? io[1] * 1000000ull / io[0] : 1000000ull;
    c->fold_on = io[0] && c->fold_sample_ppm <= FOLD_MAX_PPM;
    htrace("staged: fold sampled");
    return FK_OK;
}

static void fold_report(fk_ctx *c, bool counted) {
    uint64_t out = 0;
    for (uint32_t p : c->fold_pieces) out += c->fold_pin.as<uint64_t>()[p];
    c->fold_last[0] = counted ? c->fold_pieces.size() : 0;
    c->fold_last[1] = counted ? c->fold_in : 0;
    c->fold_last[2] = counted ? out : 0;
    c->fold_last[3] = c->fold_sample_ppm;
}

static bool fold_piece_due(const fk_ctx *c) {
    if (c->fold_mode == 2) return true;
    if (c->job_bytes && !c->piece_bytes_set) return c->st_cut == 1;
    return true;
}

static int fold_piece(fk_ctx *c, StreamWs on, uint32_t p, uint64_t pk) {
    if (pk == 0 || pk >= (1ull << 32)) return FK_OK;
    const SortedPlan &pl = c->st_plan;
    const uint64_t ncell_all = (uint64_t)c->nlb << pl.F;
    FK_TRY(ensure(c->fold_cnt, ncell_all * 4));
    FK_TRY(ensure(c->fold_cb, (ncell_all + 1) * 8));
    HIP_TRY(launch_fold_sc(c->st_keys[p].as<uint64_t>(), c->st_cb[p].as<uint64_t>(), c->nlb, c->cfg.k, pl.F, pl.F2,
                           c->fold_wmax, c->mid.as<uint64_t>(), c->fold_cnt.as<uint32_t>(), on.s));
    HIP_TRY(scan_excl_sum_u32_to_u64(c->fold_cnt.as<uint32_t>(), c->fold_cb.as<uint64_t>(), ncell_all,
                                     c->fold_cb.as<uint64_t>() + ncell_all, *on.ws, on.s));
    HIP_TRY(launch_fold_compact(c->mid.as<uint64_t>(), c->st_cb[p].as<uint64_t>(), c->fold_cb.as<uint64_t>(),
                                c->fold_cnt.as<uint32_t>(), c->nlb, pl.F, pl.F2, c->st_keys[p].as<uint64_t>(),
                                c->st_total.as<uint64_t>(), on.s));
    if (c->fold_pin.ensure(8 * STAGE_MAXP)) return set_err(FK_E_NOMEM, "hipHostMalloc failed");
    HIP_TRY(hipMemcpyAsync(c->fold_pin.as<uint64_t>() + p, c->fold_cb.as<uint64_t>() + ncell_all, 8,
                           hipMemcpyDeviceToHost, on.s));
    std::swap(c->st_cb[p], c->fold_cb);
    c->fold_in += pk;
    c->fold_pieces.push_back(p);
    htrace("staged: piece folded");
    return FK_OK;
}

static int local_maybe_piece(fk_ctx *c, uint64_t tiles, hipEvent_t mapped) {
    if (!staged_eligible(c) || c->pieces_void || !local_piece_due(c, tiles)) return FK_OK;
    const StreamWs on = c->stage_on();
    hipStream_t s = on.s;
    HIP_TRY(hipStreamWaitEvent(s, mapped, 0));
    uint64_t h[4] = {0, 0, 0, 0};
    HIP_TRY(hipMemcpyAsync(h, c->counters.p, 32, hipMemcpyDeviceToHost, s));
    HIP_TRY(hipStreamSynchronize(s));
    if (h[2]) {
        c->pieces_void = true;
        return FK_OK;
    }
    const uint64_t t0 = c->tiles_counted, nt = tiles - t0;
    const RecSrc src = fused_src(c, t0, nt, nt * map_fused_tcap());
    c->tiles_counted = tiles;
    c->st_cut += 1;
    const uint32_t p = c->st_np;
    const uint64_t k0 = c->st_kmers;
    FK_TRY(staged_expand(c, on, nullptr, src,
                         c->job_bytes ? (double)(nt * fm_tile_bytes(FUSED_NT)) / (double)c->job_bytes : 0.0));
    if (c->st_np > p && fold_eligible(c)) {
        if (!c->fold_decided) FK_TRY(fold_decide(c, on, p));
        if (c->fold_on && fold_piece_due(c)) FK_TRY(fold_piece(c, on, p, c->st_kmers - k0));
    }
    HIP_TRY(hipEventRecord(c->xstage_ev, s));
    return FK_OK;
}


enum : uint64_t { XF_FINAL = 1, XF_RETRACT = 2 };

static int plan_step(uint32_t G, uint32_t L, const uint64_t *sent, const uint64_t *got, uint64_t rb, uint64_t *soff,
                     uint64_t *sbytes, uint64_t *roff, uint64_t *rbytes, bool *all_final) {
    const size_t msg = 2 * (size_t)L + 1;
    uint64_t so = 0, ro = 0;
    bool fin = true;
    for (uint32_t d = 0; d < G; ++d) {
        uint64_t ns = 0, nr = 0;
        for (uint32_t lb = 0; lb < L; ++lb) {
            ns += sent[d * msg + lb];
            nr += got[d * msg + lb];
        }
        const uint64_t fs = sent[d * msg + 2 * L], fr = got[d * msg + 2 * L];
        if ((fs | fr) & ~(XF_FINAL | XF_RETRACT)) return set_err(FK_E_INVALID, "exchange step: unknown flag bits");
        if ((fr & XF_RETRACT) && !(fr & XF_FINAL))
            return set_err(FK_E_INVALID, "exchange step: rank %u retracts outside its last piece", d);
        fin = fin && (fr & XF_FINAL);
        soff[d] = so;
        sbytes[d] = ns * rb;
        roff[d] = ro;
        rbytes[d] = nr * rb;
        so += ns * rb;
        ro += nr * rb;
    }
    *all_final = fin;
    return FK_OK;
}

FK_EXPORT int fk_exchange_plan(int32_t n_ranks, int32_t parts, const uint64_t *sent, const uint64_t *received,
                               uint64_t record_bytes, uint64_t *send_off, uint64_t *send_bytes, uint64_t *recv_off,
                               uint64_t *recv_bytes, int32_t *all_final) {
    if (n_ranks < 1 || parts < 0 || !sent || !received || !send_off || !send_bytes || !recv_off || !recv_bytes ||
        !all_final)
        return set_err(FK_E_INVALID, "bad argument");
    bool fin = false;
    FK_TRY(plan_step((uint32_t)n_ranks, (uint32_t)parts, sent, received, record_bytes, send_off, send_bytes, recv_off,
                     recv_bytes, &fin));
    *all_final = fin ? 1 : 0;
    return FK_OK;
}

static void xch_reset(fk_ctx *c) {
    c->xch = fk_ctx::Xch{};
}

static int note_held(fk_ctx *c, int rc) {
    if (rc != FK_E_NOMEM || !c) return rc;
    std::vector<std::pair<size_t, std::string>> v;
    auto add = [&](const char *name, const DevBuf &b) {
        if (b.bytes >= (64u << 20)) v.emplace_back(b.bytes, name);
    };
#define FK_HELD(b) add(#b, c->b)
    FK_HELD(fasta_own); FK_HELD(rec_hdr); FK_HELD(rec_pos); FK_HELD(rec_code); FK_HELD(records);
    FK_HELD(codes); FK_HELD(valid); FK_HELD(precs); FK_HELD(chunks); FK_HELD(lp); FK_HELD(mid);
    FK_HELD(scratch); FK_HELD(keys); FK_HELD(out_keys); FK_HELD(out_counts); FK_HELD(buckets);
    FK_HELD(flags); FK_HELD(flag_scan); FK_HELD(cell_total); FK_HELD(cell_base); FK_HELD(dense_keys);
    FK_HELD(dense_counts); FK_HELD(bucket_unique);
    FK_HELD(sp_keys); FK_HELD(sp_subs); FK_HELD(xsend); FK_HELD(xrecv);
    add("gather_keys", c->vw.gather_keys); FK_HELD(part.K); FK_HELD(part.KT); FK_HELD(dest.K); FK_HELD(dest.KT);
#undef FK_HELD
    std::vector<std::string> piece_names(STAGE_MAXP);
    for (int p = 0; p < STAGE_MAXP; ++p) {
        piece_names[p] = "st_keys[" + std::to_string(p) + "]";
        add(piece_names[p].c_str(), c->st_keys[p]);
    }
    std::sort(v.rbegin(), v.rend());
    size_t total = 0;
    for (const auto &e : v) total += e.first;
    std::string msg = g_err + "; held on the device: " + std::to_string(total >> 20) + " MiB in";
    for (size_t i = 0; i < v.size() && i < 12; ++i)
        msg += (i ? ", " : " ") + v[i].second + " " + std::to_string(v[i].first >> 20) + " MiB";
    g_err = msg;
    return rc;
}

static int comm_fail(fk_ctx *c, int rc) {
// ... 495 lines not shown
}

FK_EXPORT int fk_debug_comm_held(fk_ctx *c) {
    if (!c || !c->comm_stream) return 0;
    DeviceGuard dg_(c->device);
    const hipError_t e = hipStreamQuery(c->comm_stream);
    if (e != hipErrorNotReady) (void)hipGetLastError();
    return e == hipErrorNotReady ? 1 : 0;
}

FK_EXPORT int fk_debug_comm_release(fk_ctx *c) {
    if (!c) return set_err(FK_E_INVALID, "null ctx");
    if (c->hold_flag) __atomic_store_n(c->hold_flag, 1u, __ATOMIC_RELEASE);
    return FK_OK;
}

static int debug_wave_count(int32_t device, int32_t k, int32_t F, uint32_t c0, uint32_t c1, int32_t slots,
                            const uint64_t *keys, uint32_t n, uint64_t *out_keys, uint32_t *out_counts,
                            uint32_t *n_out, bool weighted) {
    if (!keys || !out_keys || !out_counts || !n_out || k < 1 || k > 63 || F < 1 || F > MAX_FINE_BITS || c1 <= c0 ||
        c1 > (1u << F))
        return set_err(FK_E_INVALID, "bad argument");
    const int KW = k <= 32 ? 1 : 2;
    const uint32_t cap = KW == 1 ? WAVE_BUCKET_CAP : WAVE128_BUCKET_CAP;
    if (n == 0 || n > cap) return set_err(FK_E_RANGE, "a wave bucket holds 1..%u keys", cap);
    if (slots != (int32_t)(KW == 1 ? WAVE_SLOTS : 384))
        return set_err(FK_E_INVALID, "slots: %u (k <= 32) or 384 (k > 32)", WAVE_SLOTS);
    const int sh = 2 * k - F;
    for (uint32_t i = 0; i < n; ++i) {
        const uint64_t hi = KW == 1 ? 0 : keys[2 * i];
        uint64_t lo = KW == 1 ? keys[i] : keys[2 * i + 1];
        if (weighted && KW == 1 && 2 * k <= WKEY_MAX_BITS && (lo >> (2 * k)) <= WKEY_WMAX - 1)
            lo &= (1ull << (2 * k)) - 1ull;
        const uint64_t cell = sh >= 64 ? (hi >> (sh - 64)) : (sh == 0 ? lo : ((hi << (64 - sh)) | (lo >> sh)));
        if ((KW == 1 && k < 32 && (lo >> (2 * k)) != 0) || cell < c0 || cell >= c1)
            return set_err(FK_E_RANGE, "key %u lies outside cells [%u, %u)", i, c0, c1);
    }
    DeviceGuard dg_(device);
    TempBuf dk, dok, doc, du, db;
    FK_TRY(ensure(dk, (uint64_t)n * 8 * KW));
    FK_TRY(ensure(dok, (uint64_t)n * 8 * KW));
    FK_TRY(ensure(doc, (uint64_t)n * 4));
    FK_TRY(ensure(du, 16));
    FK_TRY(ensure(db, sizeof(Bucket)));
    const Bucket b{0, n, 0, c0, c1};
    BucketSrc wsrc{dk.as<uint64_t>(), F};
    wsrc.weighted = weighted;
    int rc = FK_OK;
    hipError_t e = hipMemcpy(dk.p, keys, (uint64_t)n * 8 * KW, hipMemcpyHostToDevice);
    if (e == hipSuccess) e = hipMemcpy(db.p, &b, sizeof(Bucket), hipMemcpyHostToDevice);
    if (e == hipSuccess)
        e = KW == 1 ? launch_bucket_count64_wave(wsrc, db.as<Bucket>(), 1, k, dok.as<uint64_t>(),
                                                 doc.as<uint32_t>(), du.as<uint64_t>(), nullptr, nullptr)
                    : launch_bucket_count128_wave(BucketSrc{dk.as<uint64_t>(), F}, db.as<Bucket>(), 1, k, dok.as<uint64_t>(),
                                                  doc.as<uint32_t>(), du.as<uint64_t>(), nullptr);
    uint64_t U = 0;
    if (e == hipSuccess) e = hipMemcpy(&U, du.p, 8, hipMemcpyDeviceToHost);
    if (e == hipSuccess && U <= n) e = hipMemcpy(out_keys, dok.p, U * 8 * KW, hipMemcpyDeviceToHost);
    if (e == hipSuccess && U <= n) e = hipMemcpy(out_counts, doc.p, U * 4, hipMemcpyDeviceToHost);
    if (e != hipSuccess) rc = set_err(FK_E_DEVICE, "%s", hipGetErrorString(e));
    else if (U > n) rc = set_err(FK_E_INVALID, "bucket reported %llu distinct keys of %u", (unsigned long long)U, n);
    *n_out = (uint32_t)U;
    return rc;
}

FK_EXPORT int fk_debug_wave_count(int32_t device, int32_t k, int32_t F, uint32_t c0, uint32_t c1, int32_t slots,
                                  const uint64_t *keys, uint32_t n, uint64_t *out_keys, uint32_t *out_counts,
                                  uint32_t *n_out) {
    return debug_wave_count(device, k, F, c0, c1, slots, keys, n, out_keys, out_counts, n_out, false);
}

FK_EXPORT int fk_debug_wave_count_w(int32_t device, int32_t k, int32_t F, uint32_t c0, uint32_t c1, int32_t slots,
                                    const uint64_t *keys, uint32_t n, uint64_t *out_keys, uint32_t *out_counts,
                                    uint32_t *n_out) {
    return debug_wave_count(device, k, F, c0, c1, slots, keys, n, out_keys, out_counts, n_out, true);
}

FK_EXPORT int fk_debug_fold_stats(const fk_ctx *c, uint64_t out[4]) {
    if (!c || !out) return set_err(FK_E_INVALID, "null argument");
    std::copy(c->fold_last, c->fold_last + 4, out);
    return FK_OK;
}

FK_EXPORT int fk_debug_map_cycles(uint64_t *out16, int32_t reset) {
    if (!out16) return set_err(FK_E_INVALID, "null argument");
    const hipError_t e = map_fused_cycles(reinterpret_cast<unsigned long long *>(out16), reset != 0);
    if (e == hipErrorNotSupported) {
        (void)hipGetLastError();
        return set_err(FK_E_STATE, "phase stamps exist only in a library built with -DFK_PROBES");
    }
    HIP_TRY(e);
    return FK_OK;
}

FK_EXPORT int fk_get_stats(fk_ctx *c, fk_stats *out) {
    if (!c || !out) return set_err(FK_E_INVALID, "null argument");
    *out = c->stats;
    return FK_OK;
}


FK_EXPORT uint64_t fk_signature_slots(const fk_ctx *c) { return c ? (1ull << (2 * c->cfg.m)) + 1ull : 0ull; }

FK_EXPORT int fk_signature_counts(fk_ctx *c, void *d_counts, uint64_t n_counts) {
    if (!c || !d_counts) return set_err(FK_E_INVALID, "null argument");
    DeviceGuard dg_(c->device);
    const uint64_t slots = fk_signature_slots(c);
    if (n_counts < slots)
        return set_err(FK_E_RANGE, "signature counts hold %llu entries, need 4^m + 1 = %llu",
                       (unsigned long long)n_counts, (unsigned long long)slots);
    if (c->pm_active && !c->pm_last_seen)
        return set_err(FK_E_STATE, "fk_signature_counts inside a streamed input: finish it with fk_ingest(..., last = 1)");
    hipStream_t s = c->stream;
    const uint64_t n = c->d_fasta ? c->n_fasta : 0;
    HIP_TRY(hipMemsetAsync(d_counts, 0, slots * 8, s));
    FK_TRY(fq_finish_pending(c, n));
    if (n) {
        const uint64_t ntiles = (n + ENC_TILE - 1) / ENC_TILE;
        const uint64_t code_words = n / 16 + 2 * POS_PAD_WORDS + 512;
        const uint64_t valid_words = n / 32 + 2 * POS_PAD_WORDS + 512;
        FK_TRY(ensure(c->tile_last_nl, ntiles * 8));
        FK_TRY(ensure(c->tile_off, ntiles * 8));
        FK_TRY(ensure(c->npos_dev, 16));
        FK_TRY(ensure(c->codes, code_words * 4));
        FK_TRY(ensure(c->valid, valid_words * 4));
        HIP_TRY(hipMemsetAsync(c->codes.p, 0, code_words * 4, s));
        HIP_TRY(hipMemsetAsync(c->valid.p, 0, valid_words * 4, s));
        HIP_TRY(hipMemsetAsync(c->npos_dev.p, 0, 16, s));
        HIP_TRY(hipMemsetAsync(c->tile_last_nl.p, 0, ntiles * 8, s));
        HIP_TRY(hipMemsetAsync(c->tile_off.p, 0, ntiles * 8, s));
        HIP_TRY(launch_fasta_parse(false, c->d_fasta, n, c->tile_last_nl.as<uint64_t>(), c->tile_off.as<uint64_t>(),
                                   c->codes.as<uint32_t>(), c->valid.as<uint32_t>(), c->npos_dev.as<uint64_t>(), s));
        HIP_TRY(launch_bin_signatures(c->codes.as<uint32_t>(), c->valid.as<uint32_t>(), n, c->npos_dev.as<uint64_t>(),
                                      c->cfg.k, c->cfg.m, (unsigned long long *)d_counts, s));
    }
    HIP_TRY(hipStreamSynchronize(s));
    return FK_OK;
}

static void signature_string(uint64_t v, char out[31]) {
    static const char rep[4] = {'A', 'C', 'G', 'T'};
    for (int j = 30; j >= 0; --j) {
        out[j] = rep[v & 3u];
        v >>= 2;
    }
}

FK_EXPORT int fk_write_bin_signatures(fk_ctx *c, const void *d_counts, uint64_t n_counts, const char *out_dir) {
    if (!c || !d_counts || !out_dir) return set_err(FK_E_INVALID, "null argument");
    DeviceGuard dg_(c->device);
    const uint64_t slots = fk_signature_slots(c);
    if (n_counts < slots)
        return set_err(FK_E_RANGE, "signature counts hold %llu entries, need 4^m + 1 = %llu",
                       (unsigned long long)n_counts, (unsigned long long)slots);
    hipStream_t s = c->stream;
    const unsigned long long *counts = (const unsigned long long *)d_counts;
    TempBuf nz, pairs;
    FK_TRY(ensure(nz, 8));
    unsigned long long nnz = 0;
    HIP_TRY(hipMemsetAsync(nz.p, 0, 8, s));
    HIP_TRY(launch_sig_compact(counts, slots, nullptr, nz.as<unsigned long long>(), s));
    HIP_TRY(hipMemcpyAsync(&nnz, nz.p, 8, hipMemcpyDeviceToHost, s));
    HIP_TRY(hipStreamSynchronize(s));
    std::vector<uint64_t> h(2 * nnz);
    if (nnz) {
        FK_TRY(ensure(pairs, nnz * 16));
// ... 50 lines not shown
```

fastkmer_amd/csrc/fk_ctx.h:

```cpp
#pragma once

#include <algorithm>
#include <string>
#include <vector>

#include "../../include/fastkmer.h"
#include "fk_comm.h"
#include "fk_internal.h"

#define FK_EXPORT extern "C" __attribute__((visibility("default")))

namespace fk {
int set_err(int code, const char *fmt, ...);
int mkdir_p(const std::string &path);

#define HIP_TRY(expr)                                                                                \
    do {                                                                                             \
        hipError_t e_ = (expr);                                                                      \
        if (e_ != hipSuccess)                                                                        \
            return set_err(e_ == hipErrorOutOfMemory ? FK_E_NOMEM : FK_E_DEVICE, "%s failed: %s (%s:%d)", \
                           #expr, hipGetErrorString(e_), __FILE__, __LINE__);                        \
    } while (0)

#define FK_TRY(expr)             \
// ... 175 lines not shown
    uint64_t pm_tiles = 0;
    bool pm_last_seen = false;
    const uint8_t *d_fasta = nullptr;
    uint64_t n_fasta = 0;
    DevBuf fasta_own;
    int32_t in_format = FK_FORMAT_FASTA, fq_min_q = 0, fq_q_off = 33;
    bool job_open = false;
    bool fq_job = false;
    uint64_t fq_done = 0;
    std::vector<uint8_t> fq_tail;
    bool fq_launched = false;
    DevBuf fq_ws, fq_info;
    PinBuf fq_pin;
    bool fq_have_info = false;
    uint64_t fq_out[3] = {0, 0, UINT64_MAX};
    std::vector<hipEvent_t> fq_evs;
    size_t fq_nev = 0;

    DevBuf tile_last_nl, tile_off, npos_dev, codes, valid;
    DevBuf records, counters, sig_status, sig_kmers;
    DevBuf tcnt;
    DevBuf rec_hdr;
    DevBuf rec_pos;
    DevBuf rec_code;
    DevBuf tstat;
    DevBuf map_vslots;
    bool rec_tiled = false;
    uint64_t rec_tiles = 0;
    uint64_t nrec = 0, nkmers = 0;
    bool mapped = false;
    std::vector<uint64_t> send_counts;
    PartBufs dest, part, binhist;
    DevBuf precs, chunks, bin_chunk_begin;
    std::vector<uint32_t> h_bcb;
    DevBuf hpieces, hpiece_first, hpiece_tot;
    DevBuf chunk_nk, chunk_base, lp, cell_total, cell_base, flags, flag_scan, buckets, keys, out_keys, out_counts;
    DevBuf scratch;
    DevBuf bucket_unique, dense_off, dense_keys, dense_counts, bin_off, misc, tier_list, mid, sc_total;
    DevBuf sp_base, sp_keys, sp_subs, sp_par, sp_fb;
    DevBuf mid_fb;
    ScanWorkspace ws;
    bool have_result = false;
    uint64_t distinct = 0;
    std::vector<uint64_t> h_bin_off;
    fk_stats stats{};
    hipEvent_t ev[12] = {};
    double ms_h2d = 0.0;
    bool ev_parse = false, ev_sig = false, ev_part = false, ev_count = false;
    std::vector<hipEvent_t> seg_evs;
    std::vector<hipEvent_t> map_evs;
    std::vector<uint64_t> seg_tiles;
    PinBuf pin_up, pin_down;
    hipEvent_t pin_up_ev = nullptr;
    bool pin_up_busy = false;
    PinBuf pin_tier;
    PinBuf file_pin[2];
    hipEvent_t tier_ev = nullptr;
    bool distinct_pending = false;
    bool gapped = false, dense_ready = false;
    const uint64_t *res_keys = nullptr;
    const uint64_t *res_fs = nullptr;
    uint64_t res_nbuckets = 0;
    int res_F = 0;
    ViewBufs vw;
    hipEvent_t cmp_ev = nullptr;

    bool pieces_void = false;
    uint64_t tiles_counted = 0;
    uint64_t job_bytes = 0;
    uint64_t reserve_bytes = 0;
    size_t segs_counted = 0;
    std::vector<double> st_cuts{0.4, 0.7, 0.9};
    std::vector<double> st_cuts5{0.38, 0.64, 0.82, 0.93};
    bool cuts_env = false;
    std::vector<double> xst_cuts{0.35, 0.65, 0.84};
    uint32_t st_np = 0;
    uint32_t st_cut = 0;
    SortedPlan st_plan;
    uint64_t st_kmers = 0;
    DevBuf st_keys[STAGE_MAXP], st_cb[STAGE_MAXP], st_total, piece_starts;
    hipEvent_t st_ev[4 * STAGE_MAXP] = {};
    int fold_mode = 1;
    uint32_t fold_wmax = WKEY_WMAX;
    bool fold_decided = false, fold_on = false;
    uint64_t fold_sample_ppm = 0;
    uint64_t fold_in = 0;
    std::vector<uint32_t> fold_pieces;
    DevBuf fold_cnt, fold_cb, fold_io;
    PinBuf fold_pin;
    uint64_t fold_last[4] = {0, 0, 0, 0};

    fk::Comm *comm = nullptr;
    hipStream_t comm_stream = nullptr;
    uint32_t *hold_flag = nullptr;
    hipStream_t xstage = nullptr;
    hipEvent_t xstage_ev = nullptr;
    ScanWorkspace ws_x;
    StreamWs main_on() { return StreamWs{stream, &ws}; }
    StreamWs stage_on() { return StreamWs{xstage, &ws_x}; }
    hipEvent_t emit_ev = nullptr;
    std::vector<hipEvent_t> xev;
    uint64_t piece_bytes = 512ull << 20;
    bool piece_bytes_set = false;
    uint64_t ingest_seg = 32ull << 20;
    DevBuf xsend, xrecv;
    struct XSeg {
        uint64_t off;
        int32_t sender;
        uint64_t step;
        std::vector<uint64_t> rec, kmer;
    };
    struct Xch {
        bool open = false;
        bool sent_final = false;
        bool all_final = false;
        bool stop_pieces = false;
        uint64_t tiles_sent = 0;
        uint64_t send_used = 0, recv_used = 0;
        uint64_t pieces = 0, bytes_sent = 0, bytes_received = 0, expect_bytes = 0;
        std::vector<XSeg> segs;
    } xch;
};

inline const uint32_t *owner_table(const fk_ctx *c) { return c->custom_owners ? c->d_owner.as<uint32_t>() : nullptr; }
inline const uint32_t *local_table(const fk_ctx *c) { return c->custom_owners ? c->d_local.as<uint32_t>() : nullptr; }
inline int32_t global_bin(const fk_ctx *c, uint32_t lb) {
    return c->custom_owners ? c->h_lbin_bin[lb] : (int32_t)(c->cfg.rank + lb * c->G);
}
inline bool owns(const fk_ctx *c, int32_t b) {
    if (b < 0 || b >= c->Bc) return false;
    return c->custom_owners ? c->h_owner[b] == c->cfg.rank : (uint32_t)b % c->G == (uint32_t)c->cfg.rank;
}
inline uint32_t local_bin(const fk_ctx *c, int32_t b) { return c->custom_owners ? c->h_bin_lbin[b] : (uint32_t)b / c->G; }
inline int32_t bin_owner(const fk_ctx *c, int32_t b) {
    return c->custom_owners ? c->h_owner[b] : (int32_t)((uint32_t)b % c->G);
}
```

fastkmer_amd/csrc/fk_expand2.inc:

```

constexpr int X2_NT = 512;
constexpr int X2_L1_CAP = 16 * X2_NT;
constexpr int X2_L2_KPT = 6;
constexpr int X2_L2_CAP = X2_L2_KPT * X2_NT;
constexpr int X2_MAX_FANOUT = 512;

template <int NTH = X2_NT>
__device__ __forceinline__ uint32_t x2_scan_digits(uint32_t *s_cnt, uint32_t *s_off, uint32_t nd, uint32_t *s_tmp,
                                                   uint32_t *total) {
    const uint32_t d = threadIdx.x;
    const uint32_t c = d < nd ? s_cnt[d] : 0u;
    const int lane = d & 63, wid = d >> 6;
    const uint32_t inc = wave_incl_sum<uint32_t>(c);
    if (lane == 63) s_tmp[wid] = inc;
    __syncthreads();
    uint32_t base = 0, tot = 0;
#pragma unroll
    for (int w = 0; w < NTH / 64; ++w) {
        const uint32_t x = s_tmp[w];
        if (w < wid) base += x;
        tot += x;
    }
    if (d < nd) {
        s_off[d] = base + inc - c;
// ... 205 lines not shown
            mid[s_cur[d] + (p - s_off[d])] = kx;
        }
        __syncthreads();
        if (threadIdx.x < S) s_cur[threadIdx.x] += mine;
    }
}

constexpr int XB_NT = 1024;
constexpr int X2_L1_WIDE_F1 = 8;

__global__ __launch_bounds__(XB_NT) void k_expand_sc1024(const uint64_t *__restrict__ rec,
                                                         const Chunk *__restrict__ chunks, int k, int F, int F1,
                                                         const uint64_t *__restrict__ cell_base,
                                                         const uint32_t *__restrict__ sc_pre,
                                                         uint64_t *__restrict__ mid) {
    __shared__ uint64_t s_stage[X2_L1_CAP];
    __shared__ uint64_t s_cur[X2_MAX_FANOUT];
    __shared__ uint32_t s_cnt[X2_MAX_FANOUT], s_off[X2_MAX_FANOUT];
    __shared__ uint32_t s_tmp[XB_NT / 64];
    const uint32_t S = 1u << F1;
    const Chunk ch = chunks[blockIdx.x];
    const uint64_t *base = cell_base + ((uint64_t)ch.lbin << F);
    for (uint32_t d = threadIdx.x; d < S; d += XB_NT) {
        s_cur[d] = base[(uint64_t)d << (F - F1)] + sc_pre[(uint64_t)blockIdx.x * S + d];
        s_cnt[d] = 0;
    }
    __syncthreads();
    const int sh = 2 * k - F1;
    const int lane = threadIdx.x & 63, wid = threadIdx.x >> 6;
    RecView<2> rn;
    if (ch.rec_begin + threadIdx.x < ch.rec_end) rn.load(rec, ch.rec_begin + threadIdx.x);
    for (uint64_t r0 = ch.rec_begin; r0 < ch.rec_end; r0 += XB_NT) {
        const uint64_t i = r0 + threadIdx.x;
        int n = 0;
        uint64_t key[16];
        uint32_t idx[16];
        if (i < ch.rec_end) {
            const RecView<2> r = rn;
            n = (int)r.n;
            record_keys64(r, k, key);
        }
        if (i + XB_NT < ch.rec_end) rn.load(rec, i + XB_NT);
#pragma unroll
        for (int j = 0; j < 16; ++j)
            if (j < n) idx[j] = atomicAdd(&s_cnt[F1 ? (uint32_t)(key[j] >> sh) : 0u], 1u);
        __syncthreads();
        const uint32_t c = threadIdx.x < S ? s_cnt[threadIdx.x] : 0u;
        const uint32_t inc = wave_incl_sum<uint32_t>(c);
        if (lane == 63) s_tmp[wid] = inc;
        __syncthreads();
        uint32_t dbase = 0, total = 0;
#pragma unroll
        for (int w = 0; w < XB_NT / 64; ++w) {
            const uint32_t x = s_tmp[w];
            if (w < wid) dbase += x;
            total += x;
        }
        if (threadIdx.x < S) {
            s_off[threadIdx.x] = dbase + inc - c;
            s_cnt[threadIdx.x] = 0;
        }
        __syncthreads();
        if (total <= (uint32_t)X2_L1_CAP) {
#pragma unroll
            for (int j = 0; j < 16; ++j)
                if (j < n) s_stage[s_off[F1 ? (uint32_t)(key[j] >> sh) : 0u] + idx[j]] = key[j];
            __syncthreads();
            for (uint32_t p = threadIdx.x; p < total; p += XB_NT) {
                const uint64_t kx = s_stage[p];
                const uint32_t d = F1 ? (uint32_t)(kx >> sh) : 0u;
                mid[s_cur[d] + (p - s_off[d])] = kx;
            }
        } else {
#pragma unroll
            for (int j = 0; j < 16; ++j)
                if (j < n) mid[s_cur[F1 ? (uint32_t)(key[j] >> sh) : 0u] + idx[j]] = key[j];
        }
        __syncthreads();
        if (threadIdx.x < S) s_cur[threadIdx.x] += c;
    }
}

template <int NTH, int KPT = X2_L2_KPT, int MAXC = (NTH < X2_MAX_FANOUT ? NTH : X2_MAX_FANOUT)>
__global__ __launch_bounds__(NTH) void k_fine_sc(const uint64_t *__restrict__ mid, int k, int F, int F2,
                                                 const uint64_t *__restrict__ cell_base,
                                                 uint64_t *__restrict__ keys) {
    constexpr int CAP = KPT * NTH;
    __shared__ uint64_t s_stage[CAP];
    __shared__ uint64_t s_cur[MAXC];
    __shared__ uint32_t s_cnt[MAXC], s_off[MAXC];
    __shared__ uint32_t s_tmp[NTH / 64];
    const uint32_t C = 1u << F2;
    const uint64_t g0 = (uint64_t)blockIdx.x << F2;
    const uint64_t a = cell_base[g0], e = cell_base[g0 + C];
    if (a == e) return;
    for (uint32_t d = threadIdx.x; d < C; d += NTH) {
        s_cur[d] = cell_base[g0 + d];
        s_cnt[d] = 0;
    }
    __syncthreads();
    const int sh = 2 * k - F;
    const uint32_t dmask = C - 1u;
    for (uint64_t b0 = a; b0 < e; b0 += CAP) {
        uint64_t key[KPT];
        uint32_t idx[KPT];
#pragma unroll
        for (int j = 0; j < KPT; ++j) {
            const uint64_t i = b0 + (uint64_t)j * NTH + threadIdx.x;
            key[j] = i < e ? __builtin_nontemporal_load(&mid[i]) : 0ull;
        }
#pragma unroll
        for (int j = 0; j < KPT; ++j) {
            const uint64_t i = b0 + (uint64_t)j * NTH + threadIdx.x;
            if (i < e) idx[j] = atomicAdd(&s_cnt[(uint32_t)(key[j] >> sh) & dmask], 1u);
        }
        __syncthreads();
        uint32_t total;
        const uint32_t mine = x2_scan_digits<NTH>(s_cnt, s_off, C, s_tmp, &total);
        __syncthreads();
#pragma unroll
        for (int j = 0; j < KPT; ++j) {
            const uint64_t i = b0 + (uint64_t)j * NTH + threadIdx.x;
            if (i < e) s_stage[s_off[(uint32_t)(key[j] >> sh) & dmask] + idx[j]] = key[j];
        }
        __syncthreads();
        for (uint32_t p = threadIdx.x; p < total; p += NTH) {
            const uint64_t kx = s_stage[p];
            const uint32_t d = (uint32_t)(kx >> sh) & dmask;
            keys[s_cur[d] + (p - s_off[d])] = kx;
        }
        __syncthreads();
        if (threadIdx.x < C) s_cur[threadIdx.x] += mine;
    }
}

hipError_t launch_expand_two_level(int KW, const uint64_t *rec, const Chunk *chunks, uint32_t nchunks,
                                   uint32_t nlbins, int k, int F, int F2, const uint32_t *sc_pre,
                                   const uint64_t *cell_base, uint64_t *mid, uint64_t *keys, hipStream_t s,
                                   int l1_threads, uint64_t nkeys) {
    if (!nchunks) return hipSuccess;
    const int F1 = F - F2;
    const int kmax = KW == 1 ? 32 : 63;
    if (F2 < 0 || F1 < 0 || (1 << F1) > X2_MAX_FANOUT || (1 << F2) > X2_MAX_FANOUT || k > kmax || F > 2 * k)
        return hipErrorInvalidValue;
    const uint64_t nsc = (uint64_t)nlbins << F1;
    uint64_t *dst1 = F2 ? mid : keys;
    const int l1 = l1_threads;
    const uint64_t kpt = KW == 1 ? X2_L2_KPT : X2W_KPT2, per_sc = nsc ? nkeys / nsc : 0;
    int l2 = per_sc <= kpt * 128 ? 128 : per_sc <= kpt * 256 ? 256 : X2_NT;
    while (l2 < X2_NT && (1 << F2) > l2) l2 *= 2;
    if (KW == 1) {
        if (l1 == 1024 || (l1 == 0 && F1 >= X2_L1_WIDE_F1))
            k_expand_sc1024<<<nchunks, XB_NT, 0, s>>>(rec, chunks, k, F, F1, cell_base, sc_pre, dst1);
        else
            k_expand_sc<<<nchunks, X2_NT, 0, s>>>(rec, chunks, k, F, F1, cell_base, sc_pre, dst1);
        if (F2 && l2 == 128)
            k_fine_sc<128><<<(unsigned)nsc, 128, 0, s>>>(mid, k, F, F2, cell_base, keys);
        else if (F2 && l2 == 256)
            k_fine_sc<256><<<(unsigned)nsc, 256, 0, s>>>(mid, k, F, F2, cell_base, keys);
        else if (F2)
            k_fine_sc<X2_NT><<<(unsigned)nsc, X2_NT, 0, s>>>(mid, k, F, F2, cell_base, keys);
    } else {
        k_expand_sc128<<<nchunks, X2W_NT1, 0, s>>>(rec, chunks, k, F, F1, cell_base, sc_pre, dst1);
        if (F2 && l2 == 128)
            k_fine_sc128<128><<<(unsigned)nsc, 128, 0, s>>>(mid, k, F, F2, cell_base, keys);
        else if (F2 && l2 == 256)
            k_fine_sc128<256><<<(unsigned)nsc, 256, 0, s>>>(mid, k, F, F2, cell_base, keys);
        else if (F2)
            k_fine_sc128<X2_NT><<<(unsigned)nsc, X2_NT, 0, s>>>(mid, k, F, F2, cell_base, keys);
    }
    return hipGetLastError();
}
```

fastkmer_amd/csrc/fk_fold.inc:

```

constexpr uint32_t FOLD_HS = 2 * FOLD_HC;
constexpr int FOLD_KPT = FOLD_HC / NT;
constexpr int FOLD_SPT = FOLD_HS / NT;
constexpr uint32_t FOLD_MAXC = 64;
static_assert((FOLD_HS & (FOLD_HS - 1)) == 0 && FOLD_HC % NT == 0 && FOLD_MAXC <= NT, "fold table");

template <bool SAMPLE>
__global__ __launch_bounds__(NT) void k_fold_sc(const uint64_t *__restrict__ keys, const uint64_t *__restrict__ cb,
                                                uint64_t nsc, int k, int F, int F2, uint32_t wmax, uint32_t stride,
                                                uint64_t *__restrict__ mid, uint32_t *__restrict__ fcount,
                                                unsigned long long *io) {
    __shared__ unsigned long long s_k[FOLD_HS];
    __shared__ uint32_t s_c[FOLD_HS];
    __shared__ uint64_t s_cb[FOLD_MAXC + 1];
    __shared__ uint32_t s_cc[FOLD_MAXC], s_cp[FOLD_MAXC];
    __shared__ uint32_t s_tot;
    const uint32_t tid = threadIdx.x;
    const uint64_t sc = (uint64_t)blockIdx.x * stride;
    if (sc >= nsc) return;
    const uint32_t ncs = 1u << F2;
    const uint64_t g0 = sc << F2;
    if (tid <= ncs) s_cb[tid] = cb[g0 + tid];
    __syncthreads();
    const WKeySpec ws = wkey_spec(k);
    const int sh = 2 * k - F;
    uint64_t cursor = s_cb[0];
    unsigned long long tin = 0, tout = 0;
    for (uint32_t c = 0; c < ncs;) {
        const uint64_t b0 = s_cb[c];
        const uint32_t lane = tid & 63u;
        const bool fits = lane >= c && lane < ncs && s_cb[lane + 1] - b0 <= FOLD_HC;
        const uint64_t fm = __ballot(fits) >> c;
        const uint32_t run = ~fm ? (uint32_t)__builtin_ctzll(~fm) : 64u;
        const uint32_t e = c + (run ? run : 1u);
        const uint64_t nb = s_cb[e] - b0;
        if (nb > FOLD_HC || nb == 0) {
            if constexpr (!SAMPLE) {
                for (uint64_t i = tid; i < nb; i += NT) mid[cursor + i] = keys[b0 + i];
                if (tid >= c && tid < e) fcount[g0 + tid] = (uint32_t)(s_cb[tid + 1] - s_cb[tid]);
            }
            tin += nb, tout += nb, cursor += nb;
            c = e;
            continue;
        }
        for (uint32_t s = tid; s < FOLD_HS; s += NT) s_k[s] = EMPTY_KEY, s_c[s] = 0;
        if (tid < FOLD_MAXC) s_cc[tid] = 0;
        __syncthreads();
        uint64_t x[FOLD_KPT];
#pragma unroll
        for (int q = 0; q < FOLD_KPT; ++q) {
            const uint32_t i = q * NT + tid;
            x[q] = i < nb ? keys[b0 + i] : EMPTY_KEY;
        }
#pragma unroll
        for (int q = 0; q < FOLD_KPT; ++q) {
            if (x[q] == EMPTY_KEY) continue;
            uint32_t wt;
            const uint64_t key = wkey_split(x[q], ws, wt);
            uint32_t s = (uint32_t)((key * 0x9e3779b97f4a7c15ull) >> (64 - __builtin_ctz(FOLD_HS)));
            for (;;) {
                unsigned long long cur = s_k[s];
                if (cur == EMPTY_KEY) cur = atomicCAS(&s_k[s], EMPTY_KEY, (unsigned long long)key);
                if (cur == EMPTY_KEY || cur == key) {
                    atomicAdd(&s_c[s], wt);
                    break;
                }
                s = (s + 1) & (FOLD_HS - 1);
            }
        }
        __syncthreads();
#pragma unroll
        for (int q = 0; q < FOLD_SPT; ++q) {
            const uint32_t s = q * NT + tid;
            const unsigned long long key = s_k[s];
            if (key != EMPTY_KEY) atomicAdd(&s_cc[(uint32_t)(key >> sh) & (ncs - 1)], (s_c[s] + wmax - 1) / wmax);
        }
        __syncthreads();
        if (tid < 64) {
            const uint32_t v = tid < ncs ? s_cc[tid] : 0u;
            const uint32_t inc = wave_incl_sum<uint32_t>(v);
            s_cp[tid] = inc - v;
            if (tid == 63) s_tot = inc;
            if constexpr (!SAMPLE)
                if (tid >= c && tid < e) fcount[g0 + tid] = v;
        }
        __syncthreads();
        const uint32_t btot = s_tot;
        if constexpr (!SAMPLE) {
#pragma unroll
            for (int q = 0; q < FOLD_SPT; ++q) {
                const uint32_t s = q * NT + tid;
                const unsigned long long key = s_k[s];
                if (key == EMPTY_KEY) continue;
                const uint32_t m = s_c[s], ne = (m + wmax - 1) / wmax;
                const uint64_t at = cursor + atomicAdd(&s_cp[(uint32_t)(key >> sh) & (ncs - 1)], ne);
                for (uint32_t t = 0; t < ne; ++t) {
                    const uint32_t w = t + 1 < ne ? wmax : m - (ne - 1) * wmax;
                    mid[at + t] = key | ((uint64_t)(w - 1) << ws.wsh);
                }
            }
        }
        tin += nb, tout += btot, cursor += btot;
        c = e;
        __syncthreads();
    }
    if constexpr (SAMPLE) {
        if (tid == 0) {
            atomicAdd(&io[0], tin);
            atomicAdd(&io[1], tout);
        }
    }
}

__global__ __launch_bounds__(NT) void k_fold_compact(const uint64_t *__restrict__ mid,
                                                     const uint64_t *__restrict__ cb_raw,
                                                     const uint64_t *__restrict__ cb_new,
                                                     const uint32_t *__restrict__ fcount, int F2,
                                                     uint64_t *__restrict__ keys, uint64_t *__restrict__ total) {
    const uint32_t ncs = 1u << F2;
    const uint64_t g0 = (uint64_t)blockIdx.x << F2;
    const uint64_t src = cb_raw[g0], dst = cb_new[g0], n = cb_new[g0 + ncs] - dst;
    for (uint64_t i = threadIdx.x; i < n; i += NT) keys[dst + i] = mid[src + i];
    if (threadIdx.x < ncs) {
        const uint64_t g = g0 + threadIdx.x;
        total[g] -= (cb_raw[g + 1] - cb_raw[g]) - fcount[g];
    }
}

hipError_t launch_fold_sc(const uint64_t *keys, const uint64_t *cb, uint32_t nlbins, int k, int F, int F2,
                          uint32_t wmax, uint64_t *mid, uint32_t *fcount, hipStream_t s) {
    const uint64_t nsc = (uint64_t)nlbins << (F - F2);
    if (!nsc) return hipSuccess;
    if (F2 > 6 || 2 * k > WKEY_MAX_BITS || wmax < 1 || wmax > WKEY_WMAX || nsc > 0x7fffffffull) return hipErrorInvalidValue;
    k_fold_sc<false><<<(unsigned)nsc, NT, 0, s>>>(keys, cb, nsc, k, F, F2, wmax, 1u, mid, fcount, nullptr);
    return hipGetLastError();
}

hipError_t launch_fold_sample(const uint64_t *keys, const uint64_t *cb, uint32_t nlbins, int k, int F, int F2,
                              uint32_t wmax, uint32_t stride, unsigned long long *io, hipStream_t s) {
    const uint64_t nsc = (uint64_t)nlbins << (F - F2);
    if (!nsc) return hipSuccess;
    if (F2 > 6 || 2 * k > WKEY_MAX_BITS || wmax < 1 || wmax > WKEY_WMAX || !stride || nsc > 0x7fffffffull)
        return hipErrorInvalidValue;
    k_fold_sc<true><<<(unsigned)((nsc + stride - 1) / stride), NT, 0, s>>>(keys, cb, nsc, k, F, F2, wmax, stride, nullptr,
                                                                          nullptr, io);
    return hipGetLastError();
}

hipError_t launch_fold_compact(const uint64_t *mid, const uint64_t *cb_raw, const uint64_t *cb_new,
                               const uint32_t *fcount, uint32_t nlbins, int F, int F2, uint64_t *keys,
                               uint64_t *total, hipStream_t s) {
    const uint64_t nsc = (uint64_t)nlbins << (F - F2);
    if (!nsc) return hipSuccess;
    if (F2 > 6 || nsc > 0x7fffffffull) return hipErrorInvalidValue;
    k_fold_compact<<<(unsigned)nsc, NT, 0, s>>>(mid, cb_raw, cb_new, fcount, F2, keys, total);
    return hipGetLastError();
}
```

fastkmer_amd/csrc/fk_internal.h:

```cpp
#pragma once

#include <hip/hip_runtime.h>
#include <stdint.h>

#include "fk_common.h"

namespace fk {

constexpr int ENC_NT = 512;
constexpr int ENC_TILE = ENC_NT * 64;
constexpr int SIG_NT = 512;
constexpr int SIG_TILE = SIG_NT * 16;
constexpr int SIG_PPT = 16;
constexpr int POS_PAD_WORDS = 64;
constexpr int SORT_CAP = 4096;
constexpr int MAX_FINE_BITS = 15;

constexpr int REC_BIN_BITS = 22;
constexpr int REC_FINE_SHIFT = 26;
constexpr uint32_t REC_BIN_MASK = (1u << REC_BIN_BITS) - 1u;

struct Bucket {
    uint64_t begin;
    uint32_t n;
// ... 49 lines not shown
                                 const uint64_t *npos_dev, int k, int m, unsigned long long *counts, hipStream_t s);
hipError_t launch_sig_compact(const unsigned long long *counts, uint64_t n, uint64_t *pairs, unsigned long long *nout,
                              hipStream_t s);

bool map_fused_supported(int k, int m, uint32_t nbins);
uint64_t fm_tile_bytes(int nth);
uint64_t fm_span_bytes(int nth);
uint32_t map_fused_tcap();
hipError_t map_fused_cycles(unsigned long long *out16, bool reset);
hipError_t rank_probe_read(unsigned long long *out4, bool reset);
uint32_t map_fused_cslot();
uint32_t map_fused_vslot();
hipError_t launch_map_fused(int nth, int k, int m, const uint8_t *fa, uint64_t n, int more, uint64_t tile_begin,
                            uint64_t ntiles, FastMod fm, uint32_t *hdrs, uint16_t *pos, uint32_t *codes,
                            uint32_t *tcnt, uint32_t *tstat, unsigned long long *counters, hipStream_t s,
                            int probe = 0, uint32_t *vslots = nullptr);
hipError_t launch_tile_totals(const uint32_t *tcnt, const uint32_t *tstat, uint64_t ntiles,
                              unsigned long long *counters, hipStream_t s);

constexpr uint32_t PART_TILE = 4096;
constexpr uint32_t PART_TPC = 4;
constexpr uint32_t PART_SEG = 64;
inline uint32_t part_segments(uint32_t nwg) { return (nwg + PART_SEG - 1) / PART_SEG; }
struct RecSrc {
    const uint64_t *rec;
    const uint32_t *tcnt;
    uint64_t nrec;
    uint64_t ntiles;
    uint32_t tcap;
    uint32_t W;
    const uint32_t *hdr;
    const uint16_t *pos;
    const uint32_t *code;
    uint32_t cslot;
    uint32_t k;
};
inline RecSrc dense_src(const uint64_t *rec, uint64_t nrec, int W) {
    return RecSrc{rec, nullptr, nrec, (nrec + PART_TILE - 1) / PART_TILE, PART_TILE, (uint32_t)W,
                  nullptr, nullptr, nullptr, 0u, 0u};
}
inline RecSrc tiled_src(const uint32_t *hdr, const uint16_t *pos, const uint32_t *code, const uint32_t *tcnt,
                        uint64_t nrec, uint64_t ntiles, uint32_t tcap, uint32_t cslot, int W, int k) {
    return RecSrc{nullptr, tcnt, nrec, ntiles, tcap, (uint32_t)W, hdr, pos, code, cslot, (uint32_t)k};
}

constexpr uint32_t PART_MAX = 12288;
uint32_t part_workgroups(const RecSrc &src);
hipError_t launch_part_hist(const RecSrc &src, int mode, uint32_t G, const uint32_t *table, uint32_t nparts,
                            uint32_t *H, uint32_t *K, hipStream_t s);
hipError_t launch_part_segsum(const uint32_t *H, const uint32_t *K, uint32_t nparts, uint32_t nwg, uint64_t *T,
                              uint64_t *KT, hipStream_t s);
hipError_t launch_part_segfill(const uint32_t *H, const uint64_t *Ts, uint32_t nparts, uint32_t nwg, uint64_t *Hs,
                               hipStream_t s);
hipError_t launch_part_totals(const uint64_t *Hs, const uint64_t *Ks, uint32_t nparts, uint32_t nwg,
                              uint64_t *part_rec, uint64_t *part_kmer, uint64_t *part_off, hipStream_t s);
hipError_t launch_part_scatter(const RecSrc &src, int mode, uint32_t G, const uint32_t *table, uint32_t nparts,
                               const uint64_t *Hs, uint64_t *out, hipStream_t s);
hipError_t launch_part_hist_global(const RecSrc &src, int mode, uint32_t G, const uint32_t *table, uint32_t nparts,
                                   uint64_t *part_rec, uint64_t *part_kmer, hipStream_t s);
hipError_t launch_part_scatter_global(const RecSrc &src, int mode, uint32_t G, const uint32_t *table,
                                      uint32_t nparts, const uint64_t *part_off, uint64_t *part_cursor,
                                      uint64_t *out, hipStream_t s);

hipError_t launch_expand_hist(int W, const uint64_t *rec, const Chunk *chunks, uint32_t nchunks, int k, int F,
                              uint32_t *hist, hipStream_t s);
hipError_t launch_cell_prefix(const uint32_t *bin_chunk_begin, uint32_t nlbins, int F, uint32_t *hist,
                              uint64_t *cell_total, hipStream_t s);
hipError_t launch_expand_scatter(int W, const uint64_t *rec, const Chunk *chunks, uint32_t nchunks, int k, int F,
                                 const uint32_t *hist, const uint64_t *cell_base, uint64_t *keys, hipStream_t s);
hipError_t launch_bucket_flags(const uint64_t *cell_base, const uint64_t *cell_total, uint32_t nlbins, int F,
                               uint32_t small_cap, uint32_t group, uint32_t *flags, hipStream_t s);
hipError_t launch_bucket_write(const uint64_t *cell_base, const uint32_t *flags, const uint64_t *flag_scan,
                               uint32_t nlbins, int F, uint64_t nbuckets, uint64_t total_keys, Bucket *buckets,
                               hipStream_t s);
hipError_t launch_bucket_count64(const BucketSrc &src, const Bucket *buckets, uint64_t nbuckets, int k,
                                 uint64_t *out_keys, uint32_t *out_counts, uint64_t *bucket_unique,
                                 unsigned long long *oversize, uint32_t small_limit, int dbg_phase,
                                 const uint32_t *list, hipStream_t s, uint32_t skip_le = 0);
hipError_t launch_bucket_count64_big(const BucketSrc &src, const Bucket *buckets, uint64_t nlist, int k,
                                     uint64_t *out_keys, uint32_t *out_counts, uint64_t *bucket_unique,
                                     unsigned long long *oversize, const uint32_t *list, hipStream_t s);
constexpr int WKEY_MAX_BITS = 60;
constexpr uint32_t WKEY_WMAX = 15;
constexpr uint32_t FOLD_HC = 1024;
hipError_t launch_fold_sc(const uint64_t *keys, const uint64_t *cb, uint32_t nlbins, int k, int F, int F2,
                          uint32_t wmax, uint64_t *mid, uint32_t *fcount, hipStream_t s);
hipError_t launch_fold_sample(const uint64_t *keys, const uint64_t *cb, uint32_t nlbins, int k, int F, int F2,
                              uint32_t wmax, uint32_t stride, unsigned long long *io, hipStream_t s);
hipError_t launch_fold_compact(const uint64_t *mid, const uint64_t *cb_raw, const uint64_t *cb_new,
                               const uint32_t *fcount, uint32_t nlbins, int F, int F2, uint64_t *keys,
                               uint64_t *total, hipStream_t s);
constexpr uint32_t WAVE_BUCKET_CAP = 512;
constexpr uint32_t WAVE_SLOTS = 640;
constexpr uint32_t WAVE_MID_CAP = 1024;
constexpr uint32_t WAVE_MID_SLOTS = 1280;
constexpr uint32_t WAVE128_BUCKET_CAP = 256;
hipError_t launch_bucket_count128_wave(const BucketSrc &src, const Bucket *buckets, uint64_t nbuckets, int k,
                                       uint64_t *out_keys, uint32_t *out_counts, uint64_t *bucket_unique,
                                       hipStream_t s, bool ordered = true);
hipError_t launch_expand_two_level(int KW, const uint64_t *rec, const Chunk *chunks, uint32_t nchunks,
                                   uint32_t nlbins, int k, int F, int F2, const uint32_t *sc_pre,
                                   const uint64_t *cell_base, uint64_t *mid, uint64_t *keys, hipStream_t s,
                                   int l1_threads = 0, uint64_t nkeys = 0);
hipError_t launch_expand_hist_pieces(int KW, const uint64_t *rec, const Chunk *chunks, const uint4 *pieces,
                                     const uint32_t *first_piece, uint32_t npieces, int k, int F, int F2,
                                     uint64_t *cell_total, uint32_t *hist_sc, uint32_t *piece_tot, hipStream_t s);
hipError_t launch_expand_hist_bin(int KW, const uint64_t *rec, const Chunk *chunks, const uint32_t *bin_chunk_begin,
                                  uint32_t nlbins, int k, int F, int F2, uint64_t *cell_total, uint32_t *hist_sc,
                                  hipStream_t s);
hipError_t launch_bucket_flags_greedy(const uint64_t *cell_total, uint32_t nlbins, int F, uint32_t cap,
                                      int period_bits, uint32_t *flags, hipStream_t s);
hipError_t launch_bucket_tiers(const Bucket *buckets, uint64_t nb, uint32_t wave_cap, uint32_t block_cap,
                               uint64_t *bucket_unique, uint32_t *lists, unsigned int *counts,
                               unsigned long long *listed_keys, hipStream_t s);
hipError_t launch_bucket_count64_wave(const BucketSrc &src, const Bucket *buckets, uint64_t nbuckets, int k,
                                      uint64_t *out_keys, uint32_t *out_counts, uint64_t *bucket_unique,
                                      const uint32_t *list, hipStream_t s, bool ordered = true);
hipError_t launch_bucket_count64_parts(const BucketSrc &src, const Bucket *buckets, const uint32_t *list,
                                       uint64_t nlist, int k, uint64_t *out_keys, uint32_t *out_counts,
                                       uint64_t *bucket_unique, uint32_t *fb, unsigned int *fb_count, hipStream_t s,
                                       bool ordered);
hipError_t launch_bucket_count64_mid512(const BucketSrc &src, const Bucket *buckets, const uint32_t *list,
                                        uint64_t nlist, int k, uint64_t *out_keys, uint32_t *out_counts,
                                        uint64_t *bucket_unique, uint32_t *fb, unsigned int *fb_count, hipStream_t s,
                                        bool ordered);
hipError_t launch_bucket_count64_wave_mid(const BucketSrc &src, const Bucket *buckets, const uint32_t *list,
                                          uint64_t nlist, int k, uint64_t *out_keys, uint32_t *out_counts,
                                          uint64_t *bucket_unique, hipStream_t s, bool ordered = true);
struct SubBucket {
    uint64_t src;
    uint64_t lo;
    uint32_t n, span;
};
struct SplitParent {
    uint32_t first, nsub;
};
hipError_t launch_listed_sizes(const Bucket *buckets, const uint32_t *list0, uint32_t n0, const uint32_t *list1,
                               uint32_t n1, uint64_t *sizes, hipStream_t s,
                               bool slots = false);
hipError_t launch_bucket_split64(const BucketSrc &src, const Bucket *buckets, const uint32_t *list0, uint32_t n0,
                                 const uint32_t *list1, uint32_t n1, const uint64_t *sbase, uint64_t *skeys,
                                 SubBucket *subs, SplitParent *parents, unsigned int *counts, uint32_t *fb0,
                                 uint32_t *fb1, uint32_t block_cap, int k, int F, hipStream_t s, bool retry = false);
hipError_t launch_sub_count64_seq(const Bucket *buckets, const uint32_t *list, uint32_t nl, const SplitParent *parents,
                                  const SubBucket *subs, const uint64_t *skeys, int k, bool weighted,
                                  uint64_t *out_keys, uint32_t *out_counts, uint64_t *bucket_unique, hipStream_t s,
                                  bool ordered);
struct SubBucket128 {
    uint64_t src;
    uint64_t lo_hi, lo_lo;
    uint32_t n, span;
};
hipError_t launch_bucket_split128(const BucketSrc &src, const Bucket *buckets, const uint32_t *list, uint32_t nl,
                                  const uint64_t *sbase, uint64_t *skeys, SubBucket128 *subs, SplitParent *parents,
                                  unsigned int *counts, uint32_t *fb0, uint32_t *fb1, uint32_t block_cap, int k, int F,
                                  hipStream_t s, bool retry = false);
hipError_t launch_sub_count128_seq(const Bucket *buckets, const uint32_t *list, uint32_t nl, const SplitParent *parents,
                                   const SubBucket128 *subs, const uint64_t *skeys, uint64_t *out_keys,
                                   uint32_t *out_counts, uint64_t *bucket_unique, hipStream_t s, bool ordered);
hipError_t launch_add_u64(uint64_t *dst, const uint64_t *src, uint64_t n, bool copy, hipStream_t s);
hipError_t launch_bucket_sort(int KW, const BucketSrc &src, const Bucket *buckets, uint64_t nbuckets, int k,
                              uint64_t *out_keys, uint32_t *out_counts, uint64_t *bucket_unique,
                              unsigned long long *oversize, uint32_t small_limit, const uint32_t *list, hipStream_t s,
                              uint32_t skip_le = 0);
constexpr uint32_t WAVE128_MID_CAP = 512;
hipError_t launch_bucket_count128_wave_mid(const BucketSrc &src, const Bucket *buckets, const uint32_t *list,
                                           uint64_t nlist, int k, uint64_t *out_keys, uint32_t *out_counts,
                                           uint64_t *bucket_unique, hipStream_t s, bool ordered = true);
hipError_t launch_bucket_sort_large(int KW, const BucketSrc &src, const Bucket *buckets, uint64_t nbuckets, int k,
                                    uint64_t *scratch, uint64_t *out_keys, uint32_t *out_counts,
                                    uint64_t *bucket_unique, const uint32_t *list, hipStream_t s,
                                    unsigned long long *scratch_cursor = nullptr);
hipError_t launch_bucket_compact(int KW, const uint64_t *out_keys, const uint32_t *out_counts,
                                 const Bucket *buckets, uint64_t nbuckets, const uint64_t *dense_off,
                                 uint64_t *dense_keys, uint32_t *dense_counts, hipStream_t s);
hipError_t launch_bin_offsets(const uint64_t *flag_scan, const uint64_t *dense_off, uint32_t nlbins, int F,
                              uint64_t nbuckets, uint64_t *bin_off, hipStream_t s);

struct QueryTables {
    const uint64_t *flag_scan;
    const Bucket *buckets;
    const uint64_t *dense_off;
    const uint64_t *keys;
    const uint32_t *counts;
    const uint32_t *owner, *local;
    uint64_t nbuckets;
// ... 55 lines not shown
```

fastkmer_amd/csrc/fk_kernels.hip:

```cpp
#include <hip/hip_runtime.h>
#include <stdint.h>

#include <algorithm>
#include <limits>
#include <type_traits>

#include "fk_internal.h"

namespace fk {

constexpr int NT = 256;


template <int CTRL, int ROWM>
__device__ __forceinline__ uint32_t dpp32(uint32_t old, uint32_t v) {
    return (uint32_t)__builtin_amdgcn_update_dpp((int)old, (int)v, CTRL, ROWM, 0xf, false);
}
template <int CTRL, int ROWM, typename T>
__device__ __forceinline__ T dpp_move(T ident, T v) {
    static_assert(sizeof(T) == 4 || sizeof(T) == 8, "32- or 64-bit scan values");
    if constexpr (sizeof(T) == 4) {
        return __builtin_bit_cast(T, dpp32<CTRL, ROWM>(__builtin_bit_cast(uint32_t, ident), __builtin_bit_cast(uint32_t, v)));
    } else {
        const uint64_t i = __builtin_bit_cast(uint64_t, ident), x = __builtin_bit_cast(uint64_t, v);
// ... 195 lines not shown
        for (int i = 0; i < (int)(sizeof(TO) * SCAN_IPT / 16); ++i) reinterpret_cast<uint4 *>(out + base)[i] = u.q[i];
    } else {
#pragma unroll
        for (int i = 0; i < SCAN_IPT; ++i) {
            uint64_t idx = base + i;
            if (idx < n) out[idx] = run;
            run = op(run, v[i]);
        }
    }
    if (total && threadIdx.x == NT - 1 && blockIdx.x == gridDim.x - 1) *total = run;
}

template <typename TI, typename TO, typename Op, bool IS_MAX>
static hipError_t scan_impl(const TI *in, TO *out, uint64_t n, TO ident, TO *total, char *ws, size_t ws_bytes,
                            hipStream_t s) {
    if (n == 0) {
        if (total) return hipMemsetAsync(total, 0, sizeof(TO), s);
        return hipSuccess;
    }
    const uint64_t nb = (n + SCAN_SEG - 1) / SCAN_SEG;
    if (nb == 1) {
        k_scan_down<TI, TO, Op, IS_MAX><<<1, NT, 0, s>>>(in, out, n, (const TO *)nullptr, ident, Op(), total);
        return hipGetLastError();
    }
    if (ws_bytes < 2 * nb * sizeof(TO)) return hipErrorOutOfMemory;
    TO *sums = (TO *)ws;
    TO *sums_scan = sums + nb;
    k_scan_reduce<TI, TO, Op, IS_MAX><<<(unsigned)nb, NT, 0, s>>>(in, n, sums, ident, Op());
    hipError_t e = scan_impl<TO, TO, Op, IS_MAX>(sums, sums_scan, nb, ident, (TO *)nullptr,
                                                 (char *)(sums_scan + nb), ws_bytes - 2 * nb * sizeof(TO), s);
    if (e != hipSuccess) return e;
    k_scan_down<TI, TO, Op, IS_MAX><<<(unsigned)nb, NT, 0, s>>>(in, out, n, sums_scan, ident, Op(), total);
    return hipGetLastError();
}

static size_t scan_ws_need(uint64_t n, size_t elem) {
    size_t need = 0;
    while (n > (uint64_t)SCAN_SEG) {
        n = (n + SCAN_SEG - 1) / SCAN_SEG;
        need += 2 * n * elem;
    }
    return need + 256;
}

static hipError_t ensure_ws(ScanWorkspace &ws, size_t need) {
    if (ws.bytes >= need) return hipSuccess;
    if (ws.ptr) (void)hipFree(ws.ptr);
    ws.ptr = nullptr;
    ws.bytes = 0;
    hipError_t e = hipMalloc(&ws.ptr, need);
    if (e == hipSuccess) ws.bytes = need;
    return e;
}

hipError_t scan_excl_sum_u64(const uint64_t *in, uint64_t *out, uint64_t n, uint64_t *total, ScanWorkspace &ws,
                             hipStream_t s) {
    hipError_t e = ensure_ws(ws, scan_ws_need(n, 8));
    if (e != hipSuccess) return e;
    return scan_impl<uint64_t, uint64_t, OpSum, false>(in, out, n, (uint64_t)0, total, (char *)ws.ptr, ws.bytes, s);
}

hipError_t scan_excl_sum_u32_to_u64(const uint32_t *in, uint64_t *out, uint64_t n, uint64_t *total,
                                    ScanWorkspace &ws, hipStream_t s) {
    hipError_t e = ensure_ws(ws, scan_ws_need(n, 8));
    if (e != hipSuccess) return e;
    return scan_impl<uint32_t, uint64_t, OpSum, false>(in, out, n, (uint64_t)0, total, (char *)ws.ptr, ws.bytes, s);
}

hipError_t scan_excl_max_i64(const int64_t *in, int64_t *out, uint64_t n, ScanWorkspace &ws, hipStream_t s) {
    hipError_t e = ensure_ws(ws, scan_ws_need(n, 8));
    if (e != hipSuccess) return e;
    return scan_impl<int64_t, int64_t, OpMax, true>(in, out, n, (int64_t)-1, (int64_t *)nullptr, (char *)ws.ptr,
                                                    ws.bytes, s);
}

#include "fk_parse.inc"
#include "fk_fastq.inc"
#include "fk_signature.inc"
#include "fk_map_fused.inc"
#include "fk_records.inc"
#include "fk_partition.inc"
#include "fk_radix_rank.inc"
#include "fk_count_sorted.inc"
#include "fk_fold.inc"
#include "fk_expand2.inc"
#include "fk_sort_radix.inc"
#include "fk_compact.inc"
#include "fk_synth.inc"
#include "fk_format.inc"
#include "fk_bin_signatures.inc"
#include "fk_query.inc"
#include "fk_spectrum.inc"
#include "fk_compare.inc"
#include "fk_reads.inc"

__global__ void __launch_bounds__(64) k_hold_stream(const uint32_t *flag, uint64_t max_ticks) {
    if (threadIdx.x != 0) return;
    const uint64_t t0 = wall_clock64();
    while (__hip_atomic_load(flag, __ATOMIC_ACQUIRE, __HIP_MEMORY_SCOPE_SYSTEM) == 0u) {
        if (wall_clock64() - t0 > max_ticks) break;
        __builtin_amdgcn_s_sleep(127);
    }
}

hipError_t launch_hold_stream(const uint32_t *flag, uint64_t max_ticks, hipStream_t s) {
    hipLaunchKernelGGL(k_hold_stream, dim3(1), dim3(64), 0, s, flag, max_ticks);
    return hipGetLastError();
}
}
```

include/fastkmer.h:

```cpp
#ifndef FASTKMER_H
#define FASTKMER_H

#include <stddef.h>
#include <stdint.h>

#ifdef __cplusplus
extern "C" {
#endif

#define FK_ABI_VERSION 3

#define FK_OK 0
#define FK_E_INVALID (-1)
#define FK_E_STATE (-2)
#define FK_E_DEVICE (-3)
#define FK_E_NOMEM (-4)
#define FK_E_IO (-5)
#define FK_E_RANGE (-6)
#define FK_E_COMM (-7)

typedef struct fk_config {
    int32_t k;
    int32_t m;
    int32_t x;
// ... 85 lines not shown
int fk_set_grouped_emit(fk_ctx *ctx, int32_t enable);
int32_t fk_grouped_parts_per_rank(const fk_ctx *ctx);
int fk_map_part_counts(fk_ctx *ctx, uint64_t *records, uint64_t *kmers);
int fk_reduce_grouped(fk_ctx *ctx, const void *d_recv, uint64_t n_records, const uint64_t *seg_records,
                      const uint64_t *seg_kmers, int32_t n_seg, int32_t parts_per_seg);
int fk_finish(fk_ctx *ctx);

int fk_map_bin_kmers(fk_ctx *ctx, uint64_t *kmers_per_bin);
int fk_lpt_owners(const uint64_t *sizes, int32_t nbins, int32_t nranks, int32_t *owner);
int fk_set_bin_owners(fk_ctx *ctx, const int32_t *owner, uint64_t *send_counts);
int fk_bin_owners(const fk_ctx *ctx, int32_t *owner);

#define FK_COMM_ID_BYTES 128
int fk_comm_unique_id(uint8_t id[FK_COMM_ID_BYTES]);
int fk_comm_init(fk_ctx *ctx, const uint8_t id[FK_COMM_ID_BYTES]);
int fk_comm_init_local(fk_ctx **ctxs, int32_t n);
const char *fk_comm_transport(const fk_ctx *ctx);
int fk_comm_allreduce_u64(fk_ctx *ctx, uint64_t *v, size_t n);
int fk_balance_bins(fk_ctx *ctx, const uint8_t *sample, size_t n);
int fk_balance_bins_file(fk_ctx *ctx, const char *path, int32_t world, int32_t rank, double fraction);
int fk_exchange_plan(int32_t n_ranks, int32_t parts, const uint64_t *sent, const uint64_t *received,
                     uint64_t record_bytes, uint64_t *send_off, uint64_t *send_bytes, uint64_t *recv_off,
                     uint64_t *recv_bytes, int32_t *all_final);


int32_t fk_num_bins(const fk_ctx *ctx);
int fk_bin_sizes(fk_ctx *ctx, uint64_t *distinct_per_bin);
int fk_get_bin(fk_ctx *ctx, int32_t bin, uint64_t *keys, uint32_t *counts, size_t cap, size_t *n);
int fk_write_bins(fk_ctx *ctx, const char *out_dir);
int fk_get_stats(fk_ctx *ctx, fk_stats *out);

int fk_kmer_bin(const fk_config *cfg, const uint64_t *key, int32_t *bin);
int fk_query(fk_ctx *ctx, const uint64_t *keys, size_t n, uint32_t *counts, int32_t *bins);
int fk_query_device(fk_ctx *ctx, const void *d_keys, size_t n, void *d_counts, void *d_bins);
int fk_query_sequence(fk_ctx *ctx, const uint8_t *seq, size_t len, uint32_t *counts, size_t cap, size_t *n);

int fk_spectrum(fk_ctx *ctx, uint64_t *hist, size_t n, uint64_t *tail_kmers);
int fk_spectrum_device(fk_ctx *ctx, void *d_hist, size_t n, void *d_tail_kmers);
int fk_bin_sizes_range(fk_ctx *ctx, uint32_t min_count, uint32_t max_count, uint64_t *distinct_per_bin);
int fk_get_bin_range(fk_ctx *ctx, int32_t bin, uint32_t min_count, uint32_t max_count,
                     uint64_t *keys, uint32_t *counts, size_t cap, size_t *n);
int fk_write_bins_range(fk_ctx *ctx, const char *out_dir, uint32_t min_count, uint32_t max_count);

int fk_compare(fk_ctx *ctx, fk_ctx *other, uint64_t *matrix, size_t rows, size_t cols);
int fk_compare_device(fk_ctx *ctx, fk_ctx *other, void *d_matrix, size_t rows, size_t cols);
int fk_bin_sizes_joined(fk_ctx *ctx, fk_ctx *other, uint32_t min_count, uint32_t max_count,
                        uint32_t other_min, uint32_t other_max, uint64_t *kept_per_bin);
int fk_get_bin_joined(fk_ctx *ctx, fk_ctx *other, int32_t bin, uint32_t min_count, uint32_t max_count,
                      uint32_t other_min, uint32_t other_max, uint64_t *keys, uint32_t *counts,
                      uint32_t *other_counts, size_t cap, size_t *n);

#define FK_READ_TILE 4096
typedef struct fk_read_stat {
    uint32_t windows;
    uint32_t hits;
    uint32_t min;
    uint32_t median;
    uint32_t max;
    uint32_t reserved;
    uint64_t sum;
} fk_read_stat;
int fk_reads_csr(const uint8_t *text, size_t n, int32_t format, int32_t min_quality, int32_t quality_offset,
                 uint8_t *bases, size_t cap_bases, uint64_t *offsets, size_t cap_reads,
                 size_t *n_reads, size_t *n_bases);
int fk_read_counts_device(fk_ctx *ctx, const void *d_bases, const void *d_offsets, size_t n_reads,
                          void *d_counts, void *d_valid);
int fk_read_counts(fk_ctx *ctx, const uint8_t *bases, const uint64_t *offsets, size_t n_reads,
                   uint32_t *counts, uint8_t *valid);
int fk_read_stats_of_counts_device(fk_ctx *ctx, const void *d_counts, const void *d_valid, const void *d_offsets,
                                   size_t n_reads, uint32_t min_count, uint32_t max_count, void *d_stats);
int fk_read_stats_device(fk_ctx *ctx, const void *d_bases, const void *d_offsets, size_t n_reads,
                         uint32_t min_count, uint32_t max_count, void *d_scratch, size_t scratch_bytes, void *d_stats);
int fk_read_stats(fk_ctx *ctx, const uint8_t *bases, const uint64_t *offsets, size_t n_reads,
                  uint32_t min_count, uint32_t max_count, fk_read_stat *stats);
size_t fk_read_stats_scratch_bytes(size_t n_bases);

int fk_debug_wave_count(int32_t device, int32_t k, int32_t F, uint32_t c0, uint32_t c1, int32_t slots,
                        const uint64_t *keys, uint32_t n, uint64_t *out_keys, uint32_t *out_counts,
                        uint32_t *n_out);
int fk_debug_wave_count_w(int32_t device, int32_t k, int32_t F, uint32_t c0, uint32_t c1, int32_t slots,
                          const uint64_t *keys, uint32_t n, uint64_t *out_keys, uint32_t *out_counts,
                          uint32_t *n_out);
int fk_debug_fold_stats(const fk_ctx *ctx, uint64_t out[4]);

int fk_debug_comm_hold(fk_ctx *ctx, int32_t max_seconds);
int fk_debug_comm_release(fk_ctx *ctx);
int fk_debug_comm_held(fk_ctx *ctx);

int fk_debug_fingerprint_bits(int32_t device, int32_t bits);

int fk_debug_map_cycles(uint64_t *out16, int32_t reset);

int fk_debug_fastq_ms(fk_ctx *ctx, double *ms, uint64_t *launches);

uint64_t fk_signature_slots(const fk_ctx *ctx);
int fk_signature_counts(fk_ctx *ctx, void *d_counts, uint64_t n_counts);
int fk_write_bin_signatures(fk_ctx *ctx, const void *d_counts, uint64_t n_counts, const char *out_dir);
int fk_find_bin_signatures(fk_ctx *ctx, const char *out_dir);

#ifdef __cplusplus
}
#endif
#endif
```

Baseline: 41.47 billion bases/s.

## Fold k-mers during level-2 expand and schedule folding per piece with a cost model

```diff
diff --git a/fastkmer_amd/__init__.py b/fastkmer_amd/__init__.py
--- a/fastkmer_amd/__init__.py
+++ b/fastkmer_amd/__init__.py
@@ -180,6 +180,7 @@
         "fk_debug_wave_count_w": (ctypes.c_int, [I32, I32, I32, ctypes.c_uint32, ctypes.c_uint32, I32, P,
                                                  ctypes.c_uint32, P, P, P]),
         "fk_debug_fold_stats": (ctypes.c_int, [P, P]),
+        "fk_debug_fold_schedule": (ctypes.c_uint32, [ctypes.c_uint64, P, ctypes.c_int32]),
     }
     for name, (res, args) in sig.items():
         fn = getattr(L, name)
@@ -758,6 +759,12 @@
                 "sample_ratio": int(out[3]) / 1e6 if out[3] else None}
 
 
+def debug_fold_schedule(job_bytes: int, cuts) -> list[bool]:
+    arr = (ctypes.c_double * len(cuts))(*cuts)
+    mask = lib().fk_debug_fold_schedule(job_bytes, arr, len(cuts))
+    return [bool(mask >> i & 1) for i in range(len(cuts))]
+
+
 def debug_wave_count(keys: np.ndarray, k: int, F: int, c0: int, c1: int, slots: int, device: int = 0,
                      weighted: bool = False):
     kw = 1 if k <= 32 else 2
diff --git a/fastkmer_amd/csrc/fk_api.cpp b/fastkmer_amd/csrc/fk_api.cpp
--- a/fastkmer_amd/csrc/fk_api.cpp
+++ b/fastkmer_amd/csrc/fk_api.cpp
@@ -257,6 +257,8 @@
     if (const char *v = env("FASTKMER_FOLD")) c->fold_mode = std::clamp(atoi(v), 0, 2);
     if (const char *v = env("FASTKMER_DEBUG_FOLD_WMAX"))
         c->fold_wmax = (uint32_t)std::clamp(atoi(v), 1, (int)WKEY_WMAX);
+    if (const char *v = env("FASTKMER_DEBUG_FOLD_LIMIT"))
+        c->fold_limit = (uint32_t)std::clamp(atoi(v), 0, (int)FOLD_LIMIT);
     if (const char *v = env("FASTKMER_X2_L1")) c->x2_l1 = atoi(v);
     if (const char *v = env("FASTKMER_FUSED")) c->fused = atoi(v);
 #ifdef FK_PROBES
@@ -395,7 +397,7 @@
         if (ev) (void)hipEventDestroy(ev);
     for (int p = 0; p < STAGE_MAXP; ++p) release(c->st_keys[p]), release(c->st_cb[p]);
     release(c->st_total);
-    release(c->fold_cnt), release(c->fold_cb), release(c->fold_io);
+    release(c->fold_cnt), release(c->fold_cb), release(c->fold_io), release(c->fold_flag);
     release(c->piece_starts);
     if (c->seg_ev) (void)hipEventDestroy(c->seg_ev);
     for (auto &ev : c->h2d_ev)
@@ -626,6 +628,11 @@
 
 static int comm_fail(fk_ctx *c, int rc);
 static int note_held(fk_ctx *c, int rc);
+
+static void ingest_segments(uint64_t n, uint64_t seg, uint64_t *big, uint64_t *small_from) {
+    *big = seg * std::clamp<uint64_t>((n / 16 + seg / 2) / seg, 1, 4);
+    *small_from = n - std::min(n, std::max<uint64_t>(n / 10, 4 * seg));
+}
 
 static int ingest_impl(fk_ctx *c, const uint8_t *fasta, size_t n, int last) {
     if (!fasta && n) return set_err(FK_E_INVALID, "null argument");
@@ -706,10 +713,10 @@
     HIP_TRY(hipEventRecord(c->h2d_ev[0], cs));
     if (pinned) {
         const size_t seg = c->ingest_seg;
-        size_t big = seg * std::clamp<size_t>((n / 16 + seg / 2) / seg, 1, 4);
-        if (pieces) big = std::min(big, std::max(seg, (size_t)c->piece_bytes / 4 / seg * seg));
+        uint64_t big = 0, small_from = 0;
+        ingest_segments(n, seg, &big, &small_from);
+        if (pieces) big = std::min<uint64_t>(big, std::max(seg, (size_t)c->piece_bytes / 4 / seg * seg));
         const size_t nseg = (n + seg - 1) / seg;
-        const size_t small_from = n - std::min(n, std::max<size_t>(n / 10, 4 * seg));
         auto seg_len = [&](size_t off) { return std::min(off < small_from ? big : seg, n - off); };
         while ((c->pm_active || fq) && c->seg_evs.size() < nseg) {
             hipEvent_t e = nullptr;
@@ -1352,7 +1359,7 @@
 }
 
 static int sorted_expand(fk_ctx *c, StreamWs on, hipStream_t cut, const SortedPlan &pl, uint32_t nchunks,
-                         uint64_t total_kmers, DevBuf &keys, DevBuf &cell_base_buf) {
+                         uint64_t total_kmers, DevBuf &keys, DevBuf &cell_base_buf, bool l1_only = false) {
     hipStream_t s = on.s;
     const int k = c->cfg.k;
     const int F = pl.F, F2 = pl.F2, F1 = pl.F1;
@@ -1412,11 +1419,19 @@
         FK_TRY(ensure(c->mid, total_kmers * 8 * c->KW));
         HIP_TRY(launch_expand_two_level(c->KW, c->rsrc, c->chunks.as<Chunk>(), nchunks, c->nlb, k, F,
                                         F2, c->lp.as<uint32_t>(), cell_base, c->mid.as<uint64_t>(),
-                                        keys.as<uint64_t>(), s, c->x2_l1, total_kmers));
+                                        keys.as<uint64_t>(), s, c->x2_l1, total_kmers, l1_only ? 1 : 3));
     } else {
         HIP_TRY(launch_expand_scatter(c->W, c->rsrc, c->chunks.as<Chunk>(), nchunks, k, F,
                                       c->lp.as<uint32_t>(), cell_base, keys.as<uint64_t>(), s));
     }
+    return FK_OK;
+}
+
+static int expand_level2(fk_ctx *c, hipStream_t s, const SortedPlan &pl, uint64_t total_kmers, DevBuf &keys,
+                         DevBuf &cell_base_buf) {
+    HIP_TRY(launch_expand_two_level(c->KW, nullptr, nullptr, 0, c->nlb, c->cfg.k, pl.F, pl.F2, nullptr,
+                                    cell_base_buf.as<uint64_t>(), c->mid.as<uint64_t>(), keys.as<uint64_t>(), s,
+                                    c->x2_l1, total_kmers, 2));
     return FK_OK;
 }
 
@@ -2046,7 +2061,7 @@
 static bool staged_eligible(const fk_ctx *c) { return staged_ok(c) && c->G == 1 && !c->comm; }
 
 static int staged_expand_chunks(fk_ctx *c, StreamWs on, hipStream_t cut, uint32_t nchunks,
-                                const std::vector<uint64_t> &bkm, double frac) {
+                                const std::vector<uint64_t> &bkm, double frac, bool l1_only = false) {
     hipStream_t s = on.s;
     const uint32_t p = c->st_np;
     uint64_t pk = 0, maxb = 0;
@@ -2060,7 +2075,7 @@
     }
     SortedPlan pl = c->st_plan;
     HIP_TRY(hipEventRecord(c->st_ev[4 * p + 2], s));
-    FK_TRY(sorted_expand(c, on, cut, pl, nchunks, pk, c->st_keys[p], c->st_cb[p]));
+    FK_TRY(sorted_expand(c, on, cut, pl, nchunks, pk, c->st_keys[p], c->st_cb[p], l1_only));
     const uint64_t ncell_all = (uint64_t)c->nlb << c->st_plan.F;
     FK_TRY(ensure(c->st_total, ncell_all * 8));
     if (cut) {
@@ -2076,7 +2091,8 @@
     return FK_OK;
 }
 
-static int staged_expand(fk_ctx *c, StreamWs on, hipStream_t cut, const RecSrc &src, double frac) {
+static int staged_expand(fk_ctx *c, StreamWs on, hipStream_t cut, const RecSrc &src, double frac,
+                         bool l1_only = false) {
     const uint32_t p = c->st_np;
     if (p >= stage_maxp(c)) return set_err(FK_E_STATE, "more than %u staged pieces", stage_maxp(c));
     uint64_t nrecv = 0;
@@ -2084,7 +2100,7 @@
     std::vector<uint32_t> bcb;
     std::vector<uint64_t> bkm;
     FK_TRY(partition_src(c, on, src, nrecv, chunks, bcb, bkm, c->st_ev[4 * p], c->st_ev[4 * p + 1]));
-    return staged_expand_chunks(c, on, cut, (uint32_t)chunks.size(), bkm, frac);
+    return staged_expand_chunks(c, on, cut, (uint32_t)chunks.size(), bkm, frac, l1_only);
 }
 
 static int staged_count(fk_ctx *c, hipStream_t cut) {
@@ -2153,8 +2169,8 @@
     const uint64_t nsc = (uint64_t)c->nlb << pl.F1;
     const uint32_t stride = (uint32_t)std::max<uint64_t>(FOLD_SAMPLE_STRIDE, (nsc / FOLD_SAMPLE_MAX) | 1ull);
     HIP_TRY(hipMemsetAsync(c->fold_io.p, 0, 16, on.s));
-    HIP_TRY(launch_fold_sample(c->st_keys[p].as<uint64_t>(), c->st_cb[p].as<uint64_t>(), c->nlb, c->cfg.k, pl.F, pl.F2,
-                               c->fold_wmax, stride, c->fold_io.as<unsigned long long>(), on.s));
+    HIP_TRY(launch_fold_sample(c->mid.as<uint64_t>(), c->st_cb[p].as<uint64_t>(), c->nlb, c->cfg.k, pl.F, pl.F2,
+                               c->fold_wmax, c->fold_limit, stride, c->fold_io.as<unsigned long long>(), on.s));
     uint64_t io[2] = {0, 0};
     HIP_TRY(hipMemcpyAsync(io, c->fold_io.p, 16, hipMemcpyDeviceToHost, on.s));
     HIP_TRY(hipStreamSynchronize(on.s));
@@ -2173,25 +2189,59 @@
     c->fold_last[3] = c->fold_sample_ppm;
 }
 
+constexpr double FOLD_H2D_MS_PER_GB = 18.1;
+constexpr double FOLD_L1_MS_PER_GB = 5.6;
+constexpr double FOLD_L2_MS_PER_GB = 2.7;
+constexpr double FOLD_FOLD_MS_PER_GB = 10.6;
+constexpr double FOLD_SLACK_MS = 0.4;
+constexpr double FOLD_MAP_MS = 0.15;
+static uint32_t fold_schedule(uint64_t job_bytes, uint64_t seg, const double *cuts, size_t ncuts) {
+    const double gb = (double)job_bytes / 1e9;
+    uint64_t big = 0, small_from = 0;
+    ingest_segments(job_bytes, seg, &big, &small_from);
+    auto stream_end = [&](uint32_t m) {
+        double t = 0.0, prev = 0.0;
+        uint64_t off = 0;
+        for (size_t j = 0; j < ncuts; ++j) {
+            const uint64_t end = std::min(job_bytes, (uint64_t)(cuts[j] * (double)job_bytes));
+            while (off < end) off += std::min(off < small_from ? big : seg, job_bytes - off);
+            const double sz = (cuts[j] - prev) * gb;
+            t = std::max(t, (double)off / 1e9 * FOLD_H2D_MS_PER_GB + FOLD_MAP_MS) +
+                sz * (FOLD_L1_MS_PER_GB + (j < 32 && (m >> j & 1u) ? FOLD_FOLD_MS_PER_GB : FOLD_L2_MS_PER_GB));
+            prev = cuts[j];
+        }
+        return t;
+    };
+    const double deadline = gb * FOLD_H2D_MS_PER_GB + FOLD_SLACK_MS;
+    uint32_t mask = 0;
+    for (size_t i = 0; i < ncuts && i < 32; ++i)
+        if (stream_end(mask | 1u << i) <= std::max(deadline, stream_end(mask))) mask |= 1u << i;
+    return mask;
+}
+
 static bool fold_piece_due(const fk_ctx *c) {
     if (c->fold_mode == 2) return true;
-    if (c->job_bytes && !c->piece_bytes_set) return c->st_cut == 1;
+    if (c->job_bytes && !c->piece_bytes_set) {
+        const std::vector<double> &cuts = local_cuts(c);
+        return c->st_cut >= 1 && c->st_cut <= 32 &&
+               (fold_schedule(c->job_bytes, c->ingest_seg, cuts.data(), cuts.size()) >> (c->st_cut - 1) & 1u);
+    }
     return true;
 }
 
 static int fold_piece(fk_ctx *c, StreamWs on, uint32_t p, uint64_t pk) {
-    if (pk == 0 || pk >= (1ull << 32)) return FK_OK;
     const SortedPlan &pl = c->st_plan;
     const uint64_t ncell_all = (uint64_t)c->nlb << pl.F;
     FK_TRY(ensure(c->fold_cnt, ncell_all * 4));
     FK_TRY(ensure(c->fold_cb, (ncell_all + 1) * 8));
-    HIP_TRY(launch_fold_sc(c->st_keys[p].as<uint64_t>(), c->st_cb[p].as<uint64_t>(), c->nlb, c->cfg.k, pl.F, pl.F2,
-                           c->fold_wmax, c->mid.as<uint64_t>(), c->fold_cnt.as<uint32_t>(), on.s));
+    FK_TRY(ensure(c->fold_flag, (uint64_t)c->nlb << pl.F1));
+    HIP_TRY(launch_fine_fold(c->mid.as<uint64_t>(), c->st_cb[p].as<uint64_t>(), c->nlb, c->cfg.k, pl.F, pl.F2,
+                             c->fold_wmax, c->fold_limit, c->fold_cnt.as<uint32_t>(), c->fold_flag.as<uint8_t>(), on.s));
     HIP_TRY(scan_excl_sum_u32_to_u64(c->fold_cnt.as<uint32_t>(), c->fold_cb.as<uint64_t>(), ncell_all,
                                      c->fold_cb.as<uint64_t>() + ncell_all, *on.ws, on.s));
     HIP_TRY(launch_fold_compact(c->mid.as<uint64_t>(), c->st_cb[p].as<uint64_t>(), c->fold_cb.as<uint64_t>(),
-                                c->fold_cnt.as<uint32_t>(), c->nlb, pl.F, pl.F2, c->st_keys[p].as<uint64_t>(),
-                                c->st_total.as<uint64_t>(), on.s));
+                                c->fold_cnt.as<uint32_t>(), c->fold_flag.as<uint8_t>(), c->nlb, c->cfg.k, pl.F, pl.F2,
+                                c->st_keys[p].as<uint64_t>(), c->st_total.as<uint64_t>(), on.s));
     if (c->fold_pin.ensure(8 * STAGE_MAXP)) return set_err(FK_E_NOMEM, "hipHostMalloc failed");
     HIP_TRY(hipMemcpyAsync(c->fold_pin.as<uint64_t>() + p, c->fold_cb.as<uint64_t>() + ncell_all, 8,
                            hipMemcpyDeviceToHost, on.s));
@@ -2220,11 +2270,16 @@
     c->st_cut += 1;
     const uint32_t p = c->st_np;
     const uint64_t k0 = c->st_kmers;
+    const bool may_fold = fold_eligible(c) && (c->fold_decided ? c->fold_on : true) && fold_piece_due(c);
     FK_TRY(staged_expand(c, on, nullptr, src,
-                         c->job_bytes ? (double)(nt * fm_tile_bytes(FUSED_NT)) / (double)c->job_bytes : 0.0));
-    if (c->st_np > p && fold_eligible(c)) {
+                         c->job_bytes ? (double)(nt * fm_tile_bytes(FUSED_NT)) / (double)c->job_bytes : 0.0, may_fold));
+    if (c->st_np > p && may_fold) {
+        const uint64_t pk = c->st_kmers - k0;
         if (!c->fold_decided) FK_TRY(fold_decide(c, on, p));
-        if (c->fold_on && fold_piece_due(c)) FK_TRY(fold_piece(c, on, p, c->st_kmers - k0));
+        if (c->fold_on && pk < (1ull << 32))
+            FK_TRY(fold_piece(c, on, p, pk));
+        else
+            FK_TRY(expand_level2(c, s, c->st_plan, pk, c->st_keys[p], c->st_cb[p]));
     }
     HIP_TRY(hipEventRecord(c->xstage_ev, s));
     return FK_OK;
@@ -2886,6 +2941,10 @@
     return FK_OK;
 }
 
+FK_EXPORT uint32_t fk_debug_fold_schedule(uint64_t job_bytes, const double *cuts, int32_t n_cuts) {
+    return cuts && n_cuts > 0 && job_bytes ? fold_schedule(job_bytes, INGEST_SEG_DEFAULT, cuts, (size_t)n_cuts) : 0u;
+}
+
 FK_EXPORT int fk_debug_map_cycles(uint64_t *out16, int32_t reset) {
     if (!out16) return set_err(FK_E_INVALID, "null argument");
     const hipError_t e = map_fused_cycles(reinterpret_cast<unsigned long long *>(out16), reset != 0);
diff --git a/fastkmer_amd/csrc/fk_ctx.h b/fastkmer_amd/csrc/fk_ctx.h
--- a/fastkmer_amd/csrc/fk_ctx.h
+++ b/fastkmer_amd/csrc/fk_ctx.h
@@ -281,11 +281,13 @@
     hipEvent_t st_ev[4 * STAGE_MAXP] = {};
     int fold_mode = 1;
     uint32_t fold_wmax = WKEY_WMAX;
+    uint32_t fold_limit = FOLD_LIMIT;
     bool fold_decided = false, fold_on = false;
     uint64_t fold_sample_ppm = 0;
     uint64_t fold_in = 0;
     std::vector<uint32_t> fold_pieces;
     DevBuf fold_cnt, fold_cb, fold_io;
+    DevBuf fold_flag;
     PinBuf fold_pin;
     uint64_t fold_last[4] = {0, 0, 0, 0};
 
@@ -301,7 +303,7 @@
     std::vector<hipEvent_t> xev;
     uint64_t piece_bytes = 512ull << 20;
     bool piece_bytes_set = false;
-    uint64_t ingest_seg = 32ull << 20;
+    uint64_t ingest_seg = INGEST_SEG_DEFAULT;
     DevBuf xsend, xrecv;
     struct XSeg {
         uint64_t off;
diff --git a/fastkmer_amd/csrc/fk_expand2.inc b/fastkmer_amd/csrc/fk_expand2.inc
--- a/fastkmer_amd/csrc/fk_expand2.inc
+++ b/fastkmer_amd/csrc/fk_expand2.inc
@@ -311,9 +311,9 @@
 }
 
 template <int NTH, int KPT = X2_L2_KPT, int MAXC = (NTH < X2_MAX_FANOUT ? NTH : X2_MAX_FANOUT)>
-__global__ __launch_bounds__(NTH) void k_fine_sc(const uint64_t *__restrict__ mid, int k, int F, int F2,
-                                                 const uint64_t *__restrict__ cell_base,
-                                                 uint64_t *__restrict__ keys) {
+__device__ __forceinline__ void x2_fine_run(const uint64_t *__restrict__ mid, uint64_t a, uint64_t e, int k, int F,
+                                            int F2, const uint64_t *__restrict__ dst_base,
+                                            uint64_t *__restrict__ keys) {
     constexpr int CAP = KPT * NTH;
     __shared__ uint64_t s_stage[CAP];
     __shared__ uint64_t s_cur[MAXC];
@@ -321,10 +321,9 @@
     __shared__ uint32_t s_tmp[NTH / 64];
     const uint32_t C = 1u << F2;
     const uint64_t g0 = (uint64_t)blockIdx.x << F2;
-    const uint64_t a = cell_base[g0], e = cell_base[g0 + C];
     if (a == e) return;
     for (uint32_t d = threadIdx.x; d < C; d += NTH) {
-        s_cur[d] = cell_base[g0 + d];
+        s_cur[d] = dst_base[g0 + d];
         s_cnt[d] = 0;
     }
     __syncthreads();
@@ -363,31 +362,45 @@
     }
 }
 
+template <int NTH, int KPT = X2_L2_KPT, int MAXC = (NTH < X2_MAX_FANOUT ? NTH : X2_MAX_FANOUT)>
+__global__ __launch_bounds__(NTH) void k_fine_sc(const uint64_t *__restrict__ mid, int k, int F, int F2,
+                                                 const uint64_t *__restrict__ cell_base,
+                                                 uint64_t *__restrict__ keys) {
+    const uint64_t g0 = (uint64_t)blockIdx.x << F2;
+    x2_fine_run<NTH, KPT, MAXC>(mid, cell_base[g0], cell_base[g0 + (1u << F2)], k, F, F2, cell_base, keys);
+}
+
 hipError_t launch_expand_two_level(int KW, const uint64_t *rec, const Chunk *chunks, uint32_t nchunks,
                                    uint32_t nlbins, int k, int F, int F2, const uint32_t *sc_pre,
                                    const uint64_t *cell_base, uint64_t *mid, uint64_t *keys, hipStream_t s,
-                                   int l1_threads, uint64_t nkeys) {
-    if (!nchunks) return hipSuccess;
+                                   int l1_threads, uint64_t nkeys, int levels) {
+    if (!nchunks && (levels & 1)) return hipSuccess;
     const int F1 = F - F2;
     const int kmax = KW == 1 ? 32 : 63;
     if (F2 < 0 || F1 < 0 || (1 << F1) > X2_MAX_FANOUT || (1 << F2) > X2_MAX_FANOUT || k > kmax || F > 2 * k)
         return hipErrorInvalidValue;
     const uint64_t nsc = (uint64_t)nlbins << F1;
-    uint64_t *dst1 = F2 ? mid : keys;
+    if (levels != 3 && KW != 1) return hipErrorInvalidValue;
+    uint64_t *dst1 = F2 || levels == 1 ? mid : keys;
+    const bool fine = F2 || levels == 2;
     const int l1 = l1_threads;
     const uint64_t kpt = KW == 1 ? X2_L2_KPT : X2W_KPT2, per_sc = nsc ? nkeys / nsc : 0;
     int l2 = per_sc <= kpt * 128 ? 128 : per_sc <= kpt * 256 ? 256 : X2_NT;
     while (l2 < X2_NT && (1 << F2) > l2) l2 *= 2;
     if (KW == 1) {
-        if (l1 == 1024 || (l1 == 0 && F1 >= X2_L1_WIDE_F1))
+        if (!(levels & 1))
+            ;
+        else if (l1 == 1024 || (l1 == 0 && F1 >= X2_L1_WIDE_F1))
             k_expand_sc1024<<<nchunks, XB_NT, 0, s>>>(rec, chunks, k, F, F1, cell_base, sc_pre, dst1);
         else
             k_expand_sc<<<nchunks, X2_NT, 0, s>>>(rec, chunks, k, F, F1, cell_base, sc_pre, dst1);
-        if (F2 && l2 == 128)
+        if (!(levels & 2) || !fine || !nsc)
+            ;
+        else if (l2 == 128)
             k_fine_sc<128><<<(unsigned)nsc, 128, 0, s>>>(mid, k, F, F2, cell_base, keys);
-        else if (F2 && l2 == 256)
+        else if (l2 == 256)
             k_fine_sc<256><<<(unsigned)nsc, 256, 0, s>>>(mid, k, F, F2, cell_base, keys);
-        else if (F2)
+        else
             k_fine_sc<X2_NT><<<(unsigned)nsc, X2_NT, 0, s>>>(mid, k, F, F2, cell_base, keys);
     } else {
         k_expand_sc128<<<nchunks, X2W_NT1, 0, s>>>(rec, chunks, k, F, F1, cell_base, sc_pre, dst1);
diff --git a/fastkmer_amd/csrc/fk_fold.inc b/fastkmer_amd/csrc/fk_fold.inc
--- a/fastkmer_amd/csrc/fk_fold.inc
+++ b/fastkmer_amd/csrc/fk_fold.inc
@@ -1,113 +1,132 @@
 
-constexpr uint32_t FOLD_HS = 2 * FOLD_HC;
-constexpr int FOLD_KPT = FOLD_HC / NT;
-constexpr int FOLD_SPT = FOLD_HS / NT;
+constexpr int FF_NT = 512;
+constexpr uint32_t FF_HS = 6144;
+constexpr int FF_KPT = 2;
+constexpr uint32_t FF_SPT = FF_HS / FF_NT;
 constexpr uint32_t FOLD_MAXC = 64;
-static_assert((FOLD_HS & (FOLD_HS - 1)) == 0 && FOLD_HC % NT == 0 && FOLD_MAXC <= NT, "fold table");
+static_assert(FOLD_ROUND == FF_KPT * FF_NT && FF_HS % FF_NT == 0 && FOLD_MAXC <= FF_NT, "fold table");
+static_assert(FOLD_LIMIT + FOLD_ROUND <= FF_HS, "fold table");
+
+__device__ __forceinline__ uint32_t ff_slot(uint64_t key) {
+    return (uint32_t)((((key * 0x9e3779b97f4a7c15ull) >> 32) * FF_HS) >> 32);
+}
 
 template <bool SAMPLE>
-__global__ __launch_bounds__(NT) void k_fold_sc(const uint64_t *__restrict__ keys, const uint64_t *__restrict__ cb,
-                                                uint64_t nsc, int k, int F, int F2, uint32_t wmax, uint32_t stride,
-                                                uint64_t *__restrict__ mid, uint32_t *__restrict__ fcount,
-                                                unsigned long long *io) {
-    __shared__ unsigned long long s_k[FOLD_HS];
-    __shared__ uint32_t s_c[FOLD_HS];
-    __shared__ uint64_t s_cb[FOLD_MAXC + 1];
+__global__ __launch_bounds__(FF_NT) void k_fine_fold(uint64_t *mid, const uint64_t *__restrict__ cb, uint64_t nsc,
+                                                     int k, int F, int F2, uint32_t wmax, uint32_t limit,
+                                                     uint32_t stride, uint32_t *__restrict__ fcount,
+                                                     uint8_t *__restrict__ unfolded, unsigned long long *io) {
+    __shared__ unsigned long long s_k[FF_HS];
+    __shared__ uint32_t s_c[FF_HS];
     __shared__ uint32_t s_cc[FOLD_MAXC], s_cp[FOLD_MAXC];
+    __shared__ uint32_t s_w[2][FF_NT / 64];
     __shared__ uint32_t s_tot;
     const uint32_t tid = threadIdx.x;
     const uint64_t sc = (uint64_t)blockIdx.x * stride;
     if (sc >= nsc) return;
     const uint32_t ncs = 1u << F2;
     const uint64_t g0 = sc << F2;
-    if (tid <= ncs) s_cb[tid] = cb[g0 + tid];
+    const uint64_t a = cb[g0], e = cb[g0 + ncs], n = e - a;
+    if (n == 0) {
+        if constexpr (!SAMPLE) {
+            if (tid < ncs) fcount[g0 + tid] = 0;
+            if (tid == 0) unfolded[sc] = 0;
+        }
+        return;
+    }
+    for (uint32_t s = tid; s < FF_HS; s += FF_NT) s_k[s] = EMPTY_KEY, s_c[s] = 0;
+    if (tid < FOLD_MAXC) s_cc[tid] = 0;
     __syncthreads();
     const WKeySpec ws = wkey_spec(k);
     const int sh = 2 * k - F;
-    uint64_t cursor = s_cb[0];
-    unsigned long long tin = 0, tout = 0;
-    for (uint32_t c = 0; c < ncs;) {
-        const uint64_t b0 = s_cb[c];
-        const uint32_t lane = tid & 63u;
-        const bool fits = lane >= c && lane < ncs && s_cb[lane + 1] - b0 <= FOLD_HC;
-        const uint64_t fm = __ballot(fits) >> c;
-        const uint32_t run = ~fm ? (uint32_t)__builtin_ctzll(~fm) : 64u;
-        const uint32_t e = c + (run ? run : 1u);
-        const uint64_t nb = s_cb[e] - b0;
-        if (nb > FOLD_HC || nb == 0) {
-            if constexpr (!SAMPLE) {
-                for (uint64_t i = tid; i < nb; i += NT) mid[cursor + i] = keys[b0 + i];
-                if (tid >= c && tid < e) fcount[g0 + tid] = (uint32_t)(s_cb[tid + 1] - s_cb[tid]);
+    uint32_t claimed = 0;
+    bool over = false;
+    uint32_t par = 0;
+    for (uint64_t b0 = a; b0 < e; b0 += FOLD_ROUND, par ^= 1u) {
+        if (claimed >= limit) {
+            over = true;
+            break;
+        }
+        uint64_t x[FF_KPT];
+#pragma unroll
+        for (int q = 0; q < FF_KPT; ++q) {
+            const uint64_t i = b0 + (uint32_t)q * FF_NT + tid;
+            x[q] = i < e ? mid[i] : EMPTY_KEY;
+        }
+        uint32_t wnew = 0;
+#pragma unroll
+        for (int q = 0; q < FF_KPT; ++q) {
+            bool mine = false;
+            if (x[q] != EMPTY_KEY) {
+                const unsigned long long key = x[q];
+                uint32_t s = ff_slot(key);
+                for (;;) {
+                    unsigned long long cur = s_k[s];
+                    if (cur == EMPTY_KEY) {
+                        cur = atomicCAS(&s_k[s], EMPTY_KEY, key);
+                        mine = cur == EMPTY_KEY;
+                    }
+                    if (cur == EMPTY_KEY || cur == key) {
+                        atomicAdd(&s_c[s], 1u);
+                        break;
+                    }
+                    s = s + 1 == FF_HS ? 0u : s + 1;
+                }
             }
-            tin += nb, tout += nb, cursor += nb;
-            c = e;
-            continue;
+            wnew += (uint32_t)__popcll(__ballot(mine));
         }
-        for (uint32_t s = tid; s < FOLD_HS; s += NT) s_k[s] = EMPTY_KEY, s_c[s] = 0;
-        if (tid < FOLD_MAXC) s_cc[tid] = 0;
-        __syncthreads();
-        uint64_t x[FOLD_KPT];
-#pragma unroll
-        for (int q = 0; q < FOLD_KPT; ++q) {
-            const uint32_t i = q * NT + tid;
-            x[q] = i < nb ? keys[b0 + i] : EMPTY_KEY;
-        }
-#pragma unroll
-        for (int q = 0; q < FOLD_KPT; ++q) {
-            if (x[q] == EMPTY_KEY) continue;
-            uint32_t wt;
-            const uint64_t key = wkey_split(x[q], ws, wt);
-            uint32_t s = (uint32_t)((key * 0x9e3779b97f4a7c15ull) >> (64 - __builtin_ctz(FOLD_HS)));
-            for (;;) {
-                unsigned long long cur = s_k[s];
-                if (cur == EMPTY_KEY) cur = atomicCAS(&s_k[s], EMPTY_KEY, (unsigned long long)key);
-                if (cur == EMPTY_KEY || cur == key) {
-                    atomicAdd(&s_c[s], wt);
-                    break;
-                }
-                s = (s + 1) & (FOLD_HS - 1);
-            }
-        }
+        if ((tid & 63u) == 0) s_w[par][tid >> 6] = wnew;
         __syncthreads();
 #pragma unroll
-        for (int q = 0; q < FOLD_SPT; ++q) {
-            const uint32_t s = q * NT + tid;
-            const unsigned long long key = s_k[s];
-            if (key != EMPTY_KEY) atomicAdd(&s_cc[(uint32_t)(key >> sh) & (ncs - 1)], (s_c[s] + wmax - 1) / wmax);
+        for (int w = 0; w < FF_NT / 64; ++w) claimed += s_w[par][w];
+    }
+    if (over) {
+        if constexpr (SAMPLE) {
+            if (tid == 0) {
+                atomicAdd(&io[0], (unsigned long long)n);
+                atomicAdd(&io[1], (unsigned long long)n);
+            }
+        } else {
+            if (tid < ncs) fcount[g0 + tid] = (uint32_t)(cb[g0 + tid + 1] - cb[g0 + tid]);
+            if (tid == 0) unfolded[sc] = 1;
         }
-        __syncthreads();
-        if (tid < 64) {
-            const uint32_t v = tid < ncs ? s_cc[tid] : 0u;
-            const uint32_t inc = wave_incl_sum<uint32_t>(v);
-            s_cp[tid] = inc - v;
-            if (tid == 63) s_tot = inc;
-            if constexpr (!SAMPLE)
-                if (tid >= c && tid < e) fcount[g0 + tid] = v;
+        return;
+    }
+#pragma unroll
+    for (uint32_t q = 0; q < FF_SPT; ++q) {
+        const uint32_t s = q * FF_NT + tid;
+        const unsigned long long key = s_k[s];
+        if (key != EMPTY_KEY) atomicAdd(&s_cc[(uint32_t)(key >> sh) & (ncs - 1)], (s_c[s] + wmax - 1) / wmax);
+    }
+    __syncthreads();
+    if (tid < 64) {
+        const uint32_t v = tid < ncs ? s_cc[tid] : 0u;
+        const uint32_t inc = wave_incl_sum<uint32_t>(v);
+        s_cp[tid] = inc - v;
+        if (tid == 63) s_tot = inc;
+        if constexpr (!SAMPLE) {
+            if (tid < ncs) fcount[g0 + tid] = v;
+            if (tid == 0) unfolded[sc] = 0;
         }
-        __syncthreads();
-        const uint32_t btot = s_tot;
-        if constexpr (!SAMPLE) {
-#pragma unroll
-            for (int q = 0; q < FOLD_SPT; ++q) {
-                const uint32_t s = q * NT + tid;
-                const unsigned long long key = s_k[s];
-                if (key == EMPTY_KEY) continue;
-                const uint32_t m = s_c[s], ne = (m + wmax - 1) / wmax;
-                const uint64_t at = cursor + atomicAdd(&s_cp[(uint32_t)(key >> sh) & (ncs - 1)], ne);
-                for (uint32_t t = 0; t < ne; ++t) {
-                    const uint32_t w = t + 1 < ne ? wmax : m - (ne - 1) * wmax;
-                    mid[at + t] = key | ((uint64_t)(w - 1) << ws.wsh);
-                }
-            }
-        }
-        tin += nb, tout += btot, cursor += btot;
-        c = e;
-        __syncthreads();
     }
+    __syncthreads();
     if constexpr (SAMPLE) {
         if (tid == 0) {
-            atomicAdd(&io[0], tin);
-            atomicAdd(&io[1], tout);
+            atomicAdd(&io[0], (unsigned long long)n);
+            atomicAdd(&io[1], (unsigned long long)s_tot);
+        }
+    } else {
+#pragma unroll
+        for (uint32_t q = 0; q < FF_SPT; ++q) {
+            const uint32_t s = q * FF_NT + tid;
+            const unsigned long long key = s_k[s];
+            if (key == EMPTY_KEY) continue;
+            const uint32_t m = s_c[s], ne = (m + wmax - 1) / wmax;
+            const uint64_t at = a + atomicAdd(&s_cp[(uint32_t)(key >> sh) & (ncs - 1)], ne);
+            for (uint32_t t = 0; t < ne; ++t) {
+                const uint32_t w = t + 1 < ne ? wmax : m - (ne - 1) * wmax;
+                mid[at + t] = key | ((uint64_t)(w - 1) << ws.wsh);
+            }
         }
     }
 }
@@ -115,10 +134,15 @@
 __global__ __launch_bounds__(NT) void k_fold_compact(const uint64_t *__restrict__ mid,
                                                      const uint64_t *__restrict__ cb_raw,
                                                      const uint64_t *__restrict__ cb_new,
-                                                     const uint32_t *__restrict__ fcount, int F2,
+                                                     const uint32_t *__restrict__ fcount,
+                                                     const uint8_t *__restrict__ unfolded, int k, int F, int F2,
                                                      uint64_t *__restrict__ keys, uint64_t *__restrict__ total) {
     const uint32_t ncs = 1u << F2;
     const uint64_t g0 = (uint64_t)blockIdx.x << F2;
+    if (unfolded[blockIdx.x]) {
+        x2_fine_run<NT>(mid, cb_raw[g0], cb_raw[g0 + ncs], k, F, F2, cb_new, keys);
+        return;
+    }
     const uint64_t src = cb_raw[g0], dst = cb_new[g0], n = cb_new[g0 + ncs] - dst;
     for (uint64_t i = threadIdx.x; i < n; i += NT) keys[dst + i] = mid[src + i];
     if (threadIdx.x < ncs) {
@@ -127,32 +151,36 @@
     }
 }
 
-hipError_t launch_fold_sc(const uint64_t *keys, const uint64_t *cb, uint32_t nlbins, int k, int F, int F2,
-                          uint32_t wmax, uint64_t *mid, uint32_t *fcount, hipStream_t s) {
+static bool fold_args_ok(uint64_t nsc, int k, int F2, uint32_t wmax, uint32_t limit) {
+    return F2 <= 6 && 2 * k <= WKEY_MAX_BITS && wmax >= 1 && wmax <= WKEY_WMAX && limit <= FOLD_LIMIT &&
+           nsc <= 0x7fffffffull;
+}
+
+hipError_t launch_fine_fold(uint64_t *mid, const uint64_t *cb, uint32_t nlbins, int k, int F, int F2, uint32_t wmax,
+                            uint32_t limit, uint32_t *fcount, uint8_t *unfolded, hipStream_t s) {
     const uint64_t nsc = (uint64_t)nlbins << (F - F2);
     if (!nsc) return hipSuccess;
-    if (F2 > 6 || 2 * k > WKEY_MAX_BITS || wmax < 1 || wmax > WKEY_WMAX || nsc > 0x7fffffffull) return hipErrorInvalidValue;
-    k_fold_sc<false><<<(unsigned)nsc, NT, 0, s>>>(keys, cb, nsc, k, F, F2, wmax, 1u, mid, fcount, nullptr);
+    if (!fold_args_ok(nsc, k, F2, wmax, limit)) return hipErrorInvalidValue;
+    k_fine_fold<false><<<(unsigned)nsc, FF_NT, 0, s>>>(mid, cb, nsc, k, F, F2, wmax, limit, 1u, fcount, unfolded, nullptr);
     return hipGetLastError();
 }
 
-hipError_t launch_fold_sample(const uint64_t *keys, const uint64_t *cb, uint32_t nlbins, int k, int F, int F2,
-                              uint32_t wmax, uint32_t stride, unsigned long long *io, hipStream_t s) {
+hipError_t launch_fold_sample(uint64_t *mid, const uint64_t *cb, uint32_t nlbins, int k, int F, int F2,
+                              uint32_t wmax, uint32_t limit, uint32_t stride, unsigned long long *io, hipStream_t s) {
     const uint64_t nsc = (uint64_t)nlbins << (F - F2);
     if (!nsc) return hipSuccess;
-    if (F2 > 6 || 2 * k > WKEY_MAX_BITS || wmax < 1 || wmax > WKEY_WMAX || !stride || nsc > 0x7fffffffull)
-        return hipErrorInvalidValue;
-    k_fold_sc<true><<<(unsigned)((nsc + stride - 1) / stride), NT, 0, s>>>(keys, cb, nsc, k, F, F2, wmax, stride, nullptr,
-                                                                          nullptr, io);
+    if (!fold_args_ok(nsc, k, F2, wmax, limit) || !stride) return hipErrorInvalidValue;
+    k_fine_fold<true><<<(unsigned)((nsc + stride - 1) / stride), FF_NT, 0, s>>>(mid, cb, nsc, k, F, F2, wmax, limit,
+                                                                               stride, nullptr, nullptr, io);
     return hipGetLastError();
 }
 
 hipError_t launch_fold_compact(const uint64_t *mid, const uint64_t *cb_raw, const uint64_t *cb_new,
-                               const uint32_t *fcount, uint32_t nlbins, int F, int F2, uint64_t *keys,
-                               uint64_t *total, hipStream_t s) {
+                               const uint32_t *fcount, const uint8_t *unfolded, uint32_t nlbins, int k, int F, int F2,
+                               uint64_t *keys, uint64_t *total, hipStream_t s) {
     const uint64_t nsc = (uint64_t)nlbins << (F - F2);
     if (!nsc) return hipSuccess;
     if (F2 > 6 || nsc > 0x7fffffffull) return hipErrorInvalidValue;
-    k_fold_compact<<<(unsigned)nsc, NT, 0, s>>>(mid, cb_raw, cb_new, fcount, F2, keys, total);
+    k_fold_compact<<<(unsigned)nsc, NT, 0, s>>>(mid, cb_raw, cb_new, fcount, unfolded, k, F, F2, keys, total);
     return hipGetLastError();
 }
diff --git a/fastkmer_amd/csrc/fk_internal.h b/fastkmer_amd/csrc/fk_internal.h
--- a/fastkmer_amd/csrc/fk_internal.h
+++ b/fastkmer_amd/csrc/fk_internal.h
@@ -155,14 +155,16 @@
                                      unsigned long long *oversize, const uint32_t *list, hipStream_t s);
 constexpr int WKEY_MAX_BITS = 60;
 constexpr uint32_t WKEY_WMAX = 15;
-constexpr uint32_t FOLD_HC = 1024;
-hipError_t launch_fold_sc(const uint64_t *keys, const uint64_t *cb, uint32_t nlbins, int k, int F, int F2,
-                          uint32_t wmax, uint64_t *mid, uint32_t *fcount, hipStream_t s);
-hipError_t launch_fold_sample(const uint64_t *keys, const uint64_t *cb, uint32_t nlbins, int k, int F, int F2,
-                              uint32_t wmax, uint32_t stride, unsigned long long *io, hipStream_t s);
+constexpr uint64_t INGEST_SEG_DEFAULT = 32ull << 20;
+constexpr uint32_t FOLD_ROUND = 1024;
+constexpr uint32_t FOLD_LIMIT = 4608;
+hipError_t launch_fine_fold(uint64_t *mid, const uint64_t *cb, uint32_t nlbins, int k, int F, int F2, uint32_t wmax,
+                            uint32_t limit, uint32_t *fcount, uint8_t *unfolded, hipStream_t s);
+hipError_t launch_fold_sample(uint64_t *mid, const uint64_t *cb, uint32_t nlbins, int k, int F, int F2,
+                              uint32_t wmax, uint32_t limit, uint32_t stride, unsigned long long *io, hipStream_t s);
 hipError_t launch_fold_compact(const uint64_t *mid, const uint64_t *cb_raw, const uint64_t *cb_new,
-                               const uint32_t *fcount, uint32_t nlbins, int F, int F2, uint64_t *keys,
-                               uint64_t *total, hipStream_t s);
+                               const uint32_t *fcount, const uint8_t *unfolded, uint32_t nlbins, int k, int F, int F2,
+                               uint64_t *keys, uint64_t *total, hipStream_t s);
 constexpr uint32_t WAVE_BUCKET_CAP = 512;
 constexpr uint32_t WAVE_SLOTS = 640;
 constexpr uint32_t WAVE_MID_CAP = 1024;
@@ -174,7 +176,7 @@
 hipError_t launch_expand_two_level(int KW, const uint64_t *rec, const Chunk *chunks, uint32_t nchunks,
                                    uint32_t nlbins, int k, int F, int F2, const uint32_t *sc_pre,
                                    const uint64_t *cell_base, uint64_t *mid, uint64_t *keys, hipStream_t s,
-                                   int l1_threads = 0, uint64_t nkeys = 0);
+                                   int l1_threads = 0, uint64_t nkeys = 0, int levels = 3);
 hipError_t launch_expand_hist_pieces(int KW, const uint64_t *rec, const Chunk *chunks, const uint4 *pieces,
                                      const uint32_t *first_piece, uint32_t npieces, int k, int F, int F2,
                                      uint64_t *cell_total, uint32_t *hist_sc, uint32_t *piece_tot, hipStream_t s);
diff --git a/fastkmer_amd/csrc/fk_kernels.hip b/fastkmer_amd/csrc/fk_kernels.hip
--- a/fastkmer_amd/csrc/fk_kernels.hip
+++ b/fastkmer_amd/csrc/fk_kernels.hip
@@ -301,8 +301,8 @@
 #include "fk_partition.inc"
 #include "fk_radix_rank.inc"
 #include "fk_count_sorted.inc"
+#include "fk_expand2.inc"
 #include "fk_fold.inc"
-#include "fk_expand2.inc"
 #include "fk_sort_radix.inc"
 #include "fk_compact.inc"
 #include "fk_synth.inc"
diff --git a/include/fastkmer.h b/include/fastkmer.h
--- a/include/fastkmer.h
+++ b/include/fastkmer.h
@@ -191,6 +191,7 @@
                           const uint64_t *keys, uint32_t n, uint64_t *out_keys, uint32_t *out_counts,
                           uint32_t *n_out);
 int fk_debug_fold_stats(const fk_ctx *ctx, uint64_t out[4]);
+uint32_t fk_debug_fold_schedule(uint64_t job_bytes, const double *cuts, int32_t n_cuts);
 
 int fk_debug_comm_hold(fk_ctx *ctx, int32_t max_seconds);
 int fk_debug_comm_release(fk_ctx *ctx);
```

Result: no change. 41.47 billion bases/s (median of 2 runs) (-0.0%).
